# ClimateImpactLab/climate_toolbox

Measured on AMD Instinct MI355X. Metric: gridcell-region-timesteps/sec, higher is better.
Workload: dtype f32

## Files before the change

### climate_toolbox_amd/_lib.py

```python
from __future__ import annotations

import ctypes as C
import os

_HERE = os.path.dirname(os.path.abspath(__file__))
LIB_PATH = os.path.join(_HERE, "lib", "libwagg.so")

EKEY, EINTERNAL = -6, -7
PLAN_NO_LC, PLAN_NO_STREAM, PLAN_NO_LINES, PLAN_LC_MFMA, PLAN_SERIAL_BUILD = 1, 2, 4, 8, 16
FORM_FULL, FORM_TILES, FORM_ENTRIES = 0, 1, 2
FORCE_FORM = {None: 0, "auto": 0, "full": 1, "tiles": 2, "entries": 3}
HOST_PIN, HOST_WHOLE, HOST_LINES, HOST_LINES_WHOLE = 1, 2, 4, 8
DENSE_GENERAL_SORT = 16
GATHER_AUTO, GATHER_RCCL, GATHER_PEER = 0, 1, 2
LAYOUT_TG, LAYOUT_GT = 0, 1
OUT_TR, OUT_RT = 0, 1

EXPORTS = (
    "wagg_version", "wagg_device_count", "wagg_shard_rows", "wagg_last_error", "wagg_profile_enable", "wagg_profile_read",
    "wagg_profile_event_overhead",
    "wagg_resolve_cells", "wagg_backup_fill", "wagg_relabel", "wagg_factorize_i64", "wagg_factorize_bytes",
    "wagg_plan_create", "wagg_plan_destroy", "wagg_plan_get_info", "wagg_plan_get_den", "wagg_plan_status",
    "wagg_apply_f32", "wagg_apply_f64", "wagg_apply_host_f32", "wagg_apply_host_f64",
    "wagg_apply_host_ex_f32", "wagg_apply_host_ex_f64", "wagg_dense_apply_host_f32", "wagg_dense_apply_host_f64",
    "wagg_apply_poly_f32", "wagg_apply_poly_f64", "wagg_apply_edd_f32", "wagg_apply_edd_f64",
    "wagg_apply_poly_host_f32", "wagg_apply_poly_host_f64", "wagg_apply_edd_host_f32", "wagg_apply_edd_host_f64",
    "wagg_gather_f32", "wagg_gather_f64",
    "wagg_transform_poly_f32", "wagg_transform_poly_f64", "wagg_transform_edd_f32", "wagg_transform_edd_f64",
    "wagg_any_less_f32", "wagg_any_less_f64",
    "wagg_dense_create_synth", "wagg_dense_create_host", "wagg_dense_create_from_segments", "wagg_dense_create_synth_blocklocal", "wagg_dense_create_synth_sparse", "wagg_dense_get_info",
    "wagg_dense_destroy", "wagg_dense_clone", "wagg_release_scratch", "wagg_scratch_bytes", "wagg_dense_get_den", "wagg_dense_apply_f32", "wagg_dense_apply_poly_f32",
    "wagg_dense_apply_edd_f32", "wagg_dense_saw_inf",
    "wagg_dense_create_synth_f64", "wagg_dense_create_host_f64", "wagg_dense_create_from_segments_f64",
    "wagg_dense_create_synth_blocklocal_f64", "wagg_dense_apply_f64", "wagg_dense_apply_poly_f64", "wagg_dense_apply_edd_f64",
    "wagg_synth_field_f32", "wagg_synth_field_f64",
    "wagg_apply_host_multi_f32", "wagg_apply_host_multi_f64", "wagg_dense_apply_host_multi_f32", "wagg_dense_apply_host_multi_f64",
    "wagg_host_block_plan", "wagg_host_stats_read",
    "wagg_combine_planes_f32", "wagg_combine_planes_f64", "wagg_take_axis", "wagg_relayout_f32", "wagg_relayout_f64",
    "wagg_dense_create_from_csr", "wagg_dense_create_from_csr_f64", "wagg_synth_table_csr", "wagg_relayout_to_f64", "wagg_upload",
    "wagg_shard_group_create", "wagg_shard_group_destroy", "wagg_shard_group_info",
    "wagg_apply_sharded_f32", "wagg_apply_sharded_f64", "wagg_dense_apply_sharded_f32", "wagg_dense_apply_sharded_f64",
    "wagg_apply", "wagg_struct_size", "wagg_struct_ordinals", "wagg_plan_get_info_sized", "wagg_dense_get_info_sized",
    "wagg_host_stats_read_sized",
    "wagg_plan_create_many", "wagg_plan_many_info", "wagg_plan_get_den_many",
)
STRUCT_PLAN_INFO, STRUCT_DENSE_INFO, STRUCT_HOST_STATS, STRUCT_APPLY_DESC = 0, 1, 2, 3
PLAN_SEGMENT, PLAN_DENSE = 0, 1
SRC_DEVICE, SRC_HOST, SRC_HOST_MULTI, SRC_SHARDED = 0, 1, 2, 3
XF_NONE, XF_POLY, XF_EDD = 0, 1, 2
APPLY_EXACT_F32 = 0x10000
T_F32, T_F64 = 7, 8


class HostStats(C.Structure):
    _fields_ = [(k, C.c_int64) for k in ("calls", "blocks", "registered", "register_failed", "unregistered", "unregister_failed",
                                         "cleanup_failed", "staged_h2d_bytes", "staged_d2h_bytes", "direct_h2d_bytes",
                                         "direct_d2h_bytes", "lines_h2d_bytes", "lines_wait_pack_us", "lines_wait_copy_us", "blocks_retired", "found_page_locked",
                                         "watched_calls", "last_rate_permille")]


def host_stats(reset=False):
    st = HostStats()
    check(load().wagg_host_stats_read_sized(C.byref(st), C.sizeof(st), 1 if reset else 0), "wagg_host_stats_read_sized")
    return {k: int(getattr(st, k)) for k, _ in HostStats._fields_}


def host_block_plan(T, row_bytes, quantum, n_devices=1):
    b, n = C.c_int64(0), C.c_int64(0)
    check(load().wagg_host_block_plan(int(T), int(row_bytes), int(quantum), int(n_devices), C.byref(b), C.byref(n)),
          "wagg_host_block_plan")
    return int(b.value), int(n.value)


class DenseInfo(C.Structure):
    _fields_ = [("G", C.c_int64), ("n_tiles", C.c_int64), ("w_bytes", C.c_int64),
                ("R", C.c_int32), ("n_kt", C.c_int32), ("n_nt", C.c_int32), ("tiled", C.c_int32),
                ("form", C.c_int32), ("elem_bytes", C.c_int32), ("nnz", C.c_int64),
                ("build_s", C.c_double), ("build_upload_s", C.c_double),
                ("est_full_s", C.c_double), ("est_tiles_s", C.c_double), ("est_entries_s", C.c_double), ("walked_entries", C.c_int64),
                ("one_pass_sort", C.c_int32), ("reserved0", C.c_int32)]


class WaggError(RuntimeError):
    pass


class PlanInfo(C.Structure):
    _fields_ = [("nseg_in", C.c_int64), ("nnz", C.c_int64), ("n_groups", C.c_int64),
                ("n_chunks", C.c_int64), ("n_ucells", C.c_int64), ("n_giant", C.c_int64),
                ("n_empty", C.c_int64), ("G", C.c_int64), ("R", C.c_int32), ("lines", C.c_int32),
                ("n_lines128", C.c_int64), ("n_sectors64", C.c_int64), ("n_partial_rows", C.c_int64),
                ("lines_chunks", C.c_int64), ("lines_ucells", C.c_int64), ("lines_lines128", C.c_int64),
                ("n_partial_rows64", C.c_int64), ("lines64_chunks", C.c_int64), ("lines64_ucells", C.c_int64)]


class ApplyDesc(C.Structure):
    _fields_ = [("struct_size", C.c_uint64), ("plan_kind", C.c_int32), ("elem", C.c_int32), ("source", C.c_int32), ("transform", C.c_int32),
                ("plan", C.c_void_p), ("x", C.c_void_p), ("x2", C.c_void_p), ("out", C.c_void_p),
                ("T", C.c_int64), ("ldx", C.c_int64), ("ldo", C.c_int64), ("out_pstride", C.c_int64),
                ("layout", C.c_int32), ("out_layout", C.c_int32), ("offset", C.c_double), ("pow_first", C.c_int32), ("n_pow", C.c_int32),
                ("thresholds", C.c_void_p), ("n_thr", C.c_int32), ("flags", C.c_int32), ("ksplit", C.c_int32), ("n_plans", C.c_int32),
                ("devices", C.c_void_p), ("rows", C.c_void_p), ("group", C.c_void_p), ("root", C.c_int32), ("reserved0", C.c_int32),
                ("stream", C.c_void_p)]


STRUCTS = {STRUCT_PLAN_INFO: PlanInfo, STRUCT_DENSE_INFO: DenseInfo, STRUCT_HOST_STATS: HostStats, STRUCT_APPLY_DESC: ApplyDesc}


def _ptr(v):
    if v is None:
        return None
    if isinstance(v, int):
        return v
    if isinstance(v, C.c_void_p):
        return v.value
    return C.cast(v, C.c_void_p).value


def run(what, **fields):
    d = ApplyDesc()
    d.struct_size = C.sizeof(ApplyDesc)
    d.pow_first = d.n_pow = 1
    for k, v in fields.items():
        setattr(d, k, _ptr(v) if k in _DESC_POINTERS else v)
    check(load().wagg_apply(C.byref(d)), what)


_DESC_POINTERS = frozenset(k for k, t in ApplyDesc._fields_ if t is C.c_void_p)

_lib = None


def load():
    global _lib
    if _lib is not None:
        return _lib
    if not os.path.exists(LIB_PATH):
        raise WaggError(
            "HIP engine not built: %s is missing. Run `python -c \"import __graft_entry__ as g; "
            "g.build()\"` or `make -C climate_toolbox_amd/csrc`. There is no CPU fallback." % LIB_PATH)
    import torch
    L = C.CDLL(LIB_PATH)
    vp, i32p, f64p, f32p = C.c_void_p, C.POINTER(C.c_int32), C.POINTER(C.c_double), C.POINTER(C.c_float)
    L.wagg_version.restype = C.c_int
    L.wagg_shard_rows.argtypes = [C.c_int64, C.c_int, C.c_int, C.POINTER(C.c_int64), C.POINTER(C.c_int64)]
    L.wagg_device_count.restype = C.c_int
    L.wagg_last_error.restype = C.c_char_p
    L.wagg_profile_enable.argtypes = [C.c_int]
    L.wagg_profile_read.argtypes = [f32p, C.c_int, C.POINTER(C.c_int)]
    L.wagg_profile_event_overhead.argtypes = [vp, C.c_int, f32p, f32p]
    u8p, i64p = C.POINTER(C.c_uint8), C.POINTER(C.c_int64)
    L.wagg_resolve_cells.argtypes = [f64p, C.c_int64, f64p, C.c_int64, f64p, f64p, C.c_int64, C.c_int, i32p, i64p]
    L.wagg_backup_fill.argtypes = [f64p, f64p, C.c_int64, f64p]
    L.wagg_relabel.argtypes = [f64p, C.c_int64, C.c_double, C.c_double]
    L.wagg_factorize_i64.argtypes = [i64p, u8p, C.c_int64, i32p, i64p, i64p]
    L.wagg_factorize_bytes.argtypes = [C.c_char_p, C.c_int64, u8p, C.c_int64, i32p, i64p, i64p]
    L.wagg_plan_create.argtypes = [i32p, i32p, f64p, C.c_int64, C.c_int64, C.c_int32, C.c_int64,
                                   C.c_int, C.POINTER(vp)]
    L.wagg_plan_create_many.argtypes = [i32p, i32p, C.POINTER(f64p), C.c_int, C.c_int64, C.c_int64, C.c_int32, C.c_int64,
                                        C.POINTER(i32p), i32p, C.c_int, C.c_int, C.POINTER(vp)]
    L.wagg_plan_many_info.argtypes = [vp, C.POINTER(C.c_int), C.POINTER(C.c_int), i32p, i64p]
    L.wagg_plan_get_den_many.argtypes = [vp, C.c_int, C.c_int, f64p]
    L.wagg_plan_destroy.argtypes = [vp]
    L.wagg_plan_get_info.argtypes = [vp, C.POINTER(PlanInfo)]
    L.wagg_plan_get_info_sized.argtypes = [vp, vp, C.c_uint64]
    L.wagg_dense_get_info_sized.argtypes = [vp, vp, C.c_uint64]
    L.wagg_host_stats_read_sized.argtypes = [vp, C.c_uint64, C.c_int]
    L.wagg_struct_size.argtypes = [C.c_int]
    L.wagg_struct_ordinals.argtypes = [C.c_int, vp, C.c_uint64]
    L.wagg_apply.argtypes = [C.POINTER(ApplyDesc)]
    L.wagg_plan_get_den.argtypes = [vp, f64p]
    L.wagg_plan_status.argtypes = [vp, vp]
    for name in ("wagg_apply_f32", "wagg_apply_f64"):
        getattr(L, name).argtypes = [vp, vp, C.c_int64, C.c_int64, C.c_int, vp, C.c_int64, C.c_int, vp]
    for name in ("wagg_apply_poly_f32", "wagg_apply_poly_f64"):
        getattr(L, name).argtypes = [vp, vp, C.c_int64, C.c_int64, C.c_int, C.c_double, C.c_int, C.c_int, vp,
                                     C.c_int64, C.c_int64, C.c_int, vp]
    for name in ("wagg_apply_poly_host_f32", "wagg_apply_poly_host_f64"):
        getattr(L, name).argtypes = [vp, vp, C.c_int64, C.c_int64, C.c_double, C.c_int, C.c_int, vp, C.c_int64, C.c_int64, C.c_int]
    for name in ("wagg_apply_edd_host_f32", "wagg_apply_edd_host_f64"):
        getattr(L, name).argtypes = [vp, vp, vp, C.c_int64, C.c_int64, C.c_double, f64p, C.c_int, vp, C.c_int64, C.c_int64, C.c_int]
    for name in ("wagg_apply_edd_f32", "wagg_apply_edd_f64"):
        getattr(L, name).argtypes = [vp, vp, vp, C.c_int64, C.c_int64, C.c_int, C.c_double, f64p, C.c_int, vp,
                                     C.c_int64, C.c_int64, C.c_int, vp]
    for name in ("wagg_apply_host_f32", "wagg_apply_host_f64"):
        getattr(L, name).argtypes = [vp, vp, C.c_int64, C.c_int64, C.c_int, vp, C.c_int64, C.c_int]
    for name in ("wagg_apply_host_ex_f32", "wagg_apply_host_ex_f64"):
        getattr(L, name).argtypes = [vp, vp, C.c_int64, C.c_int64, C.c_int, vp, C.c_int64, C.c_int, C.c_int]
    for name in ("wagg_dense_apply_host_f32", "wagg_dense_apply_host_f64"):
        getattr(L, name).argtypes = [vp, vp, C.c_int64, C.c_int64, vp, C.c_int64, C.c_int]
    for name in ("wagg_apply_host_multi_f32", "wagg_apply_host_multi_f64", "wagg_dense_apply_host_multi_f32",
                 "wagg_dense_apply_host_multi_f64"):
        getattr(L, name).argtypes = [C.POINTER(vp), i32p, C.c_int, vp, C.c_int64, C.c_int64, vp, C.c_int64, C.c_int]
    for name in ("wagg_combine_planes_f32", "wagg_combine_planes_f64"):
        getattr(L, name).argtypes = [vp, C.c_int, C.c_int64, f64p, C.c_int64, vp, vp]
    L.wagg_take_axis.argtypes = [vp, C.c_int64, C.c_int64, C.c_int64, vp, C.c_int64, vp, vp]
    for name in ("wagg_relayout_f32", "wagg_relayout_f64"):
        getattr(L, name).argtypes = [vp, C.c_int, C.POINTER(C.c_int64), C.POINTER(C.c_int64), vp, vp]
    L.wagg_relayout_to_f64.argtypes = [vp, C.c_int, C.c_int, C.POINTER(C.c_int64), C.POINTER(C.c_int64), vp, vp]
    L.wagg_upload.argtypes = [vp, vp, C.c_int64]
    L.wagg_host_block_plan.argtypes = [C.c_int64, C.c_int64, C.c_int64, C.c_int, C.POINTER(C.c_int64), C.POINTER(C.c_int64)]
    L.wagg_host_stats_read.argtypes = [C.POINTER(HostStats), C.c_int]
    for name in ("wagg_gather_f32", "wagg_gather_f64"):
        getattr(L, name).argtypes = [vp, C.c_int64, C.c_int64, C.c_int, vp, C.c_int64, vp, C.c_int64,
                                     C.c_int, vp]
    for name in ("wagg_transform_poly_f32", "wagg_transform_poly_f64"):
        getattr(L, name).argtypes = [vp, C.c_int64, C.c_double, C.c_int, vp, vp]
    for name in ("wagg_transform_edd_f32", "wagg_transform_edd_f64"):
        getattr(L, name).argtypes = [vp, vp, C.c_int64, C.c_double, f64p, f64p, C.c_int, vp, vp]
    for name in ("wagg_any_less_f32", "wagg_any_less_f64"):
        getattr(L, name).argtypes = [vp, vp, C.c_int64, C.POINTER(C.c_int), vp]
    L.wagg_dense_create_synth.argtypes = [C.c_int64, C.c_int32, C.c_uint32, C.POINTER(vp)]
    L.wagg_dense_create_host.argtypes = [f32p, C.c_int64, C.c_int32, C.POINTER(vp)]
    L.wagg_dense_create_from_segments.argtypes = [i32p, i32p, f64p, C.c_int64, C.c_int64, C.c_int32, C.c_int,
                                                  C.POINTER(vp)]
    L.wagg_dense_create_synth_blocklocal.argtypes = [C.c_int64, C.c_int32, C.c_uint32, C.c_double, C.POINTER(vp)]
    L.wagg_dense_create_synth_sparse.argtypes = [C.c_int64, C.c_int32, C.c_uint32, C.c_double, C.POINTER(vp)]
    L.wagg_dense_get_info.argtypes = [vp, C.POINTER(DenseInfo)]
    L.wagg_dense_destroy.argtypes = [vp]
    L.wagg_dense_clone.argtypes = [vp, C.c_int, C.POINTER(vp)]
    L.wagg_release_scratch.argtypes = []
    L.wagg_scratch_bytes.argtypes = []
    L.wagg_scratch_bytes.restype = C.c_int64
    L.wagg_dense_get_den.argtypes = [vp, f64p]
    L.wagg_dense_apply_f32.argtypes = [vp, vp, C.c_int64, C.c_int64, vp, C.c_int64, C.c_int, vp]
    L.wagg_dense_apply_poly_f32.argtypes = [vp, vp, C.c_int64, C.c_int64, C.c_double, C.c_int, vp, C.c_int64, C.c_int, vp]
    L.wagg_dense_apply_edd_f32.argtypes = [vp, vp, vp, C.c_int64, C.c_int64, C.c_double, C.c_double, vp, C.c_int64,
                                           C.c_int, vp]
    L.wagg_dense_saw_inf.argtypes = [vp, vp, C.POINTER(C.c_int)]
    L.wagg_dense_create_synth_f64.argtypes = [C.c_int64, C.c_int32, C.c_uint32, C.c_double, C.POINTER(vp)]
    L.wagg_dense_create_synth_blocklocal_f64.argtypes = [C.c_int64, C.c_int32, C.c_uint32, C.c_double, C.POINTER(vp)]
    L.wagg_dense_create_host_f64.argtypes = [f64p, C.c_int64, C.c_int32, C.POINTER(vp)]
    L.wagg_dense_create_from_segments_f64.argtypes = [i32p, i32p, f64p, C.c_int64, C.c_int64, C.c_int32, C.c_int, C.POINTER(vp)]
    for name in ("wagg_dense_create_from_csr", "wagg_dense_create_from_csr_f64"):
        getattr(L, name).argtypes = [i64p, i32p, f64p, C.c_int64, C.c_int32, C.c_int, C.POINTER(vp)]
    L.wagg_synth_table_csr.argtypes = [C.c_int64, C.c_int32, C.c_uint32, C.c_double, C.c_int, i64p, i32p, f64p, C.c_int64, i64p]
    L.wagg_dense_apply_f64.argtypes = [vp, vp, C.c_int64, C.c_int64, vp, C.c_int64, C.c_int, vp]
    L.wagg_dense_apply_poly_f64.argtypes = [vp, vp, C.c_int64, C.c_int64, C.c_double, C.c_int, vp, C.c_int64, C.c_int, vp]
    L.wagg_dense_apply_edd_f64.argtypes = [vp, vp, vp, C.c_int64, C.c_int64, C.c_double, C.c_double, vp, C.c_int64,
                                           C.c_int, vp]
    L.wagg_synth_field_f32.argtypes = [vp, C.c_int64, C.c_int64, C.c_int64, C.c_uint32, C.c_float,
                                       C.c_float, vp]
    L.wagg_synth_field_f64.argtypes = [vp, C.c_int64, C.c_int64, C.c_int64, C.c_uint32, C.c_double,
                                       C.c_double, vp]
    L.wagg_shard_group_create.argtypes = [i32p, C.c_int, C.c_int, C.POINTER(vp)]
    L.wagg_shard_group_destroy.argtypes = [vp]
    L.wagg_shard_group_info.argtypes = [vp, C.POINTER(C.c_int), C.POINTER(C.c_int)]
    for name in ("wagg_apply_sharded_f32", "wagg_apply_sharded_f64", "wagg_dense_apply_sharded_f32", "wagg_dense_apply_sharded_f64"):
        getattr(L, name).argtypes = [vp, C.POINTER(vp), C.POINTER(vp), i64p, C.c_int64, vp, C.c_int64, C.c_int]
    for name in EXPORTS:
        fn = getattr(L, name)
        if name not in ("wagg_last_error", "wagg_scratch_bytes"):
            fn.restype = C.c_int
    _lib = L
    return L


def check(rc, what):
    if rc != 0:
        msg = load().wagg_last_error().decode("utf-8", "replace")
        err = WaggError("%s failed (%d): %s" % (what, rc, msg))
        err.code = int(rc)
        raise err
```

### climate_toolbox_amd/_plans.py

```python
from __future__ import annotations

import os
import threading
from collections import OrderedDict

from ._lib import FORM_ENTRIES, WaggError
from ._memo import _CACHE_LOCK, _fingerprint
from .engine import DensePlan, SparsePlan

_PLAN_CACHE: "OrderedDict[str, SparsePlan]" = OrderedDict()
_PLAN_CACHE_MAX = 8
_PLAN_CACHE_MAX_FRAC = 0.5
_REPLICA_MAX_BYTES = 8 << 30


def _host_devices(setting):
    import torch
    HOST_DEVICES = setting
    if HOST_DEVICES is None:
        return []
    if isinstance(HOST_DEVICES, str):
        if HOST_DEVICES != "all":
            raise ValueError('HOST_DEVICES must be None, "all" or a list of device ordinals')
        if int(os.environ.get("WORLD_SIZE", "1")) > 1:
            return []
        return list(range(torch.cuda.device_count()))
    return [int(d) for d in HOST_DEVICES]


def _host_quantum(plan):
    if isinstance(plan, DensePlan):
        f64 = plan.dtype == "float64"
        if plan.info["form"] == FORM_ENTRIES:
            return 64 if f64 else 128
        return 176 if f64 else 368
    return 64


def _host_replicas(plan, n_rows, row_bytes, setting=None):
    devs = _host_devices(setting)
    if len(devs) < 2 or _plan_bytes(plan) > _REPLICA_MAX_BYTES:
        return ()
    from ._lib import host_block_plan
    if host_block_plan(n_rows, row_bytes, _host_quantum(plan), len(devs))[1] < 2 * len(devs):
        return ()
    own = devs.index(plan.device) if plan.device in devs else 0
    cache = plan.__dict__.setdefault("_replicas", {})
    out = []
    for slot, d in enumerate(devs):
        if slot == own:
            continue
        key = (slot, d)
        if key not in cache:
            cache[key] = plan.replica(d)
        out.append(cache[key])
    return tuple(out)


DENSE_SWITCH = 16.0
_SPARSE_CELLS_PER_S = {True: 2.7e11, False: 1.8e11}
_DENSE_MARGIN = 1.5
_DENSE_BUILD_BYTES_PER_ROW = 64
_ENOMEM = -3


def _dense_floor_s(G, R, nseg, is_f32):
    b = 4 if is_f32 else 8
    n_rb = -(-int(R) // (16 * 43))
    loop = 2.0 * 1.3 * float(nseg) / (30e12 if is_f32 else 13e12)
    pack = 2.0 * b * float(G) / 5.3e12
    return max(b * float(G) * n_rb / 10.1e12, loop) + pack


def _wants_dense(n_ucells, G, layout, R=None, nseg=None, is_f32=True):
    if layout != "TG":
        return False
    if R is None or nseg is None:
        return n_ucells > DENSE_SWITCH * G
    return n_ucells / _SPARSE_CELLS_PER_S[bool(is_f32)] > _DENSE_MARGIN * _dense_floor_s(G, R, nseg, is_f32)


def _dense_bytes(G, R, is_f32=True, nseg=None):
    eb = 4 if is_f32 else 8
    full = eb * ((int(G) + 31) // 32 * 32) * ((int(R) + 255) // 256 * 256)
    if nseg is not None:
        n_buckets = 16 * (-(-int(R) // 688)) * (-(-int(G) // 128))
        return min(full, (64 if is_f32 else 160) * int(nseg) + 7 * (8 if is_f32 else 16) * n_buckets)
    return full


def _prefer_dense(n_ucells, G, R, is_f32, layout, free_bytes, nseg=None):
    return (_wants_dense(n_ucells, G, layout, R=R, nseg=nseg if nseg is not None else n_ucells, is_f32=is_f32)
            and _dense_bytes(G, R, is_f32, nseg=nseg) < 0.6 * free_bytes)


def _plan_bytes(plan):
    return int(plan.info.get("w_bytes", 0)) if isinstance(plan, DensePlan) else 16 * int(plan.info.get("nnz", 0))


def _evict_plans(byte_budget, keep):
    freed = 0
    held = sum(_plan_bytes(p) for p in _PLAN_CACHE.values())
    for key in list(_PLAN_CACHE):
        if not (len(_PLAN_CACHE) > keep or held > max(byte_budget, 0)):
            break
        old = _PLAN_CACHE[key]
        if not old._lease.acquire(blocking=False):
            continue
        try:
            del _PLAN_CACHE[key]
            b = _plan_bytes(old)
            old.close()
        finally:
            old._lease.release()
        held -= b
        freed += b
    return freed


def _drop_plan(plan):
    with _CACHE_LOCK:
        for key, p in list(_PLAN_CACHE.items()):
            if p is plan:
                del _PLAN_CACHE[key]
    plan.close()


_BUILDING = {}


def _plan_for(cell_idx, codes, w_eff, G, R, row_len, is_f32=False, layout="TG", prepared=None):
    if prepared is not None:
        key = prepared.plan_key(cell_idx, G, R, row_len, is_f32, layout)
    else:
        key, _ = _fingerprint(cell_idx, codes, w_eff, extra=repr((int(G), int(R), int(row_len), bool(is_f32), layout)))
    while True:
        with _CACHE_LOCK:
            plan = _PLAN_CACHE.get(key)
            pending = None
            if plan is not None:
                _PLAN_CACHE.move_to_end(key)
            else:
                pending = _BUILDING.get(key)
                if pending is None:
                    _BUILDING[key] = threading.Event()
        if plan is not None:
            plan._lease.acquire()
            if plan._h.value:
                return plan
            plan._lease.release()
            with _CACHE_LOCK:
                if _PLAN_CACHE.get(key) is plan:
                    del _PLAN_CACHE[key]
            continue
        if pending is not None:
            pending.wait()
            continue
        break
    import torch
    plan = None
    try:
        with _CACHE_LOCK:
            free_bytes, total_bytes = torch.cuda.mem_get_info()
            from . import _lib as _libmod
            if _libmod._lib is not None:
                free_bytes += int(_libmod._lib.wagg_scratch_bytes())
            free_bytes += _evict_plans(_PLAN_CACHE_MAX_FRAC * total_bytes, keep=_PLAN_CACHE_MAX - 1)
        need = _dense_bytes(G, R, is_f32, nseg=len(cell_idx)) + _DENSE_BUILD_BYTES_PER_ROW * len(cell_idx)

        def dense_fits():
            nonlocal free_bytes
            if need >= 0.6 * free_bytes:
                with _CACHE_LOCK:
                    free_bytes += _evict_plans(_PLAN_CACHE_MAX_FRAC * total_bytes - need, keep=_PLAN_CACHE_MAX - 1)
            return need < 0.6 * free_bytes

        dt = "float32" if is_f32 else "float64"

        def dense_plan():
            if len(cell_idx) >= 2 ** 31:
                return None
            for attempt in (0, 1):
                try:
                    return DensePlan.from_segments(cell_idx, codes, w_eff, G, R, dtype=dt)
                except WaggError as e:
# ... 80 lines not shown
```

### climate_toolbox_amd/csrc/wagg_common.h

```cpp
#pragma once
#include <hip/hip_runtime.h>
#include <hip/hip_ext.h>
#include <cstdarg>
#include <cstdint>
#include <cstdio>
#include <cstring>
#include <new>
#include <vector>

#include "../../include/wagg.h"

namespace wagg {

void set_error(const char *fmt, ...);

#define WAGG_HIP(expr)                                                                        \
    do {                                                                                      \
        hipError_t e__ = (expr);                                                              \
        if (e__ != hipSuccess) {                                                              \
            wagg::set_error("%s:%d: %s -> %s", __FILE__, __LINE__, #expr,                     \
                            hipGetErrorString(e__));                                          \
            return WAGG_EHIP;                                                                 \
        }                                                                                     \
    } while (0)
// ... 41 lines not shown
    p = __builtin_fmaf(p, az, 0.0010792884277179837f);
    p = __builtin_fmaf(p, az, -0.002406827174127102f);
    p = __builtin_fmaf(p, az, 0.005977150052785873f);
    p = __builtin_fmaf(p, az, -0.022534651681780815f);
    p = __builtin_fmaf(p, az, 0.31830987334251404f);
    const float q = __builtin_amdgcn_sqrtf(t) * t;
    return __builtin_fmaf(w, q * p, __builtin_fmaxf(d, 0.0f));
}
__device__ __forceinline__ double snyder_edd1_finite(double tmin, double tmax, double e) {
    const double M = 0.5 * (tmax + tmin), w = 0.5 * (tmax - tmin);
    const double d = M - e;
    double rw = __builtin_amdgcn_rcp(w);
    rw = __builtin_fma(rw, __builtin_fma(-w, rw, 1.0), rw);
    const double az = __builtin_fmin(__builtin_fabs(d * rw), 1.0);
    const double t = 1.0 - az;
    const double ty = __builtin_amdgcn_rsq(__builtin_fmax(t, 1e-300));
    double st = t * ty;
    st = __builtin_fma(__builtin_fma(-st, st, t), 0.5 * ty, st);
    double p = -8.644295123170258e-07;
    p = __builtin_fma(p, az, 7.147532263874047e-06);
    p = __builtin_fma(p, az, -2.807399717529102e-05);
    p = __builtin_fma(p, az, 7.126284961634285e-05);
    p = __builtin_fma(p, az, -0.0001359898123558899);
    p = __builtin_fma(p, az, 0.0002182750865254441);
    p = __builtin_fma(p, az, -0.0003242640574299061);
    p = __builtin_fma(p, az, 0.000480605991421148);
    p = __builtin_fma(p, az, -0.0007477719612718598);
    p = __builtin_fma(p, az, 0.0012691227365052833);
    p = __builtin_fma(p, az, -0.0024647062510063378);
    p = __builtin_fma(p, az, 0.005985979570242935);
    p = __builtin_fma(p, az, -0.0225351707225776);
    p = __builtin_fma(p, az, 0.3183098861837864);
    return __builtin_fma(w, st * t * p, __builtin_fmax(d, 0.0));
}
template <> __device__ __forceinline__ float snyder_edd1<float>(float tmin, float tmax, float e) {
    const float d = 0.5f * (tmax + tmin) - e;
    const float inner = snyder_edd1_finite(tmin, tmax, e);
    return !(tmin < e) ? d : (!(tmax > e) ? 0.0f : inner);
}

template <typename T> __device__ __forceinline__ T xform1(T x, T off, int pw) {
    const T y = x + off;
    T r = y;
    for (int i = 1; i < pw; ++i) r *= y;
    return r;
}
template <typename V, typename T> __device__ __forceinline__ V xform4(V v, T off, int pw) {
    V r;
#pragma unroll
    for (int c = 0; c < 4; ++c) r[c] = xform1<T>(v[c], off, pw);
    return r;
}

void copy_sized(void *dst, uint64_t dst_size, const void *src, size_t src_size);

hipError_t allow_dynamic_lds(const void *kern, size_t bytes);

bool profile_slot(hipEvent_t *start, hipEvent_t *stop);

inline hipError_t launch_timed_ptr(bool timed, const void *kern, dim3 grid, dim3 block, void **args, size_t shmem, hipStream_t st) {
    hipEvent_t a = nullptr, b = nullptr;
    if (timed && profile_slot(&a, &b)) return hipExtLaunchKernel(kern, grid, block, args, shmem, st, a, b, 0);
    return hipLaunchKernel(kern, grid, block, args, shmem, st);
}
template <typename... Args, typename F = void (*)(Args...)>
inline void launch_timed(bool timed, F kern, dim3 grid, dim3 block, size_t shmem, hipStream_t st, Args... args) {
    hipEvent_t a = nullptr, b = nullptr;
    if (timed && profile_slot(&a, &b)) hipExtLaunchKernelGGL(kern, grid, block, (std::uint32_t)shmem, st, a, b, 0u, args...);
    else hipLaunchKernelGGL(kern, grid, block, shmem, st, args...);
}

hipError_t staged_h2d(void *dst_dev, const void *src_host, size_t bytes, hipStream_t st);
hipError_t staged_d2h_rows(void *dst_host, const void *src_dev, int64_t rows, size_t ld_bytes, size_t row_bytes, hipStream_t st);
inline hipError_t staged_d2h(void *dst_host, const void *src_dev, size_t bytes, hipStream_t st = nullptr) {
    return staged_d2h_rows(dst_host, src_dev, 1, bytes, bytes, st);
}
void clear_error();

hipError_t scratch_alloc(void **p, size_t bytes);
void scratch_free(void *p, bool keep = true);
hipError_t scratch_stream(hipStream_t *st, int role = 0);
void scratch_stream_done(hipStream_t st, int role = 0, bool keep = true);
void release_scratch(int what = 7);
template <typename T>
struct ScratchBuf {
    T *p = nullptr;
    ScratchBuf() = default;
    ScratchBuf(const ScratchBuf &) = delete;
    ScratchBuf &operator=(const ScratchBuf &) = delete;
    hipError_t alloc(size_t count) { return scratch_alloc(reinterpret_cast<void **>(&p), (count ? count : 1) * sizeof(T)); }
    ~ScratchBuf() { if (p) { (void)hipDeviceSynchronize(); scratch_free(p); } }
};

template <typename T>
struct DevBuf {
    T *p = nullptr;
    size_t n = 0;
    DevBuf() = default;
    DevBuf(const DevBuf &) = delete;
    DevBuf &operator=(const DevBuf &) = delete;
    ~DevBuf() { if (p) (void)hipFree(p); }
    hipError_t alloc(size_t count) {
        if (p) { (void)hipFree(p); p = nullptr; }
        n = count;
        hipError_t e = hipMalloc((void **)&p, (count ? count : 1) * sizeof(T));
        if (e == hipErrorOutOfMemory) {
            (void)hipGetLastError();
            release_scratch();
            e = hipMalloc((void **)&p, (count ? count : 1) * sizeof(T));
        }
        return e;
    }
    hipError_t upload(const std::vector<T> &h, hipStream_t st = nullptr) {
        hipError_t e = alloc(h.size());
        if (e != hipSuccess || h.empty()) return e;
        return staged_h2d(p, h.data(), h.size() * sizeof(T), st);
    }
};

}
```

### climate_toolbox_amd/csrc/wagg_dense.hip

```cpp
#include <algorithm>
#include <cfloat>
#include <chrono>
#include <cmath>
#include <limits>
#include <cstdlib>
#include <type_traits>

#include "wagg_dense_int.h"
#include "wagg_entry.h"

namespace wagg {

constexpr int D_MT = 23;
constexpr int D_BN = 256;
constexpr int D_ROWB = 128;
constexpr int D_THREADS = 512;
constexpr int D_WTB = D_BN * D_ROWB;
constexpr int D_WSLOTS = D_WTB / 16;
static_assert(D_WTB / 1024 == 32, "4 one-KiB W pieces per wave");
constexpr int d_xt_bytes(int mt) { return mt * 16 * D_ROWB; }
constexpr int d_buf_bytes(int mt) { return d_xt_bytes(mt) + D_WTB; }
static_assert(2 * d_buf_bytes(D_MT) <= 160 * 1024, "LDS budget");

typedef float f32x4 __attribute__((ext_vector_type(4)));
typedef double f64x2 __attribute__((ext_vector_type(2)));
typedef double f64x4 __attribute__((ext_vector_type(4)));
typedef const void __attribute__((address_space(1))) *gptr_t;
typedef void __attribute__((address_space(3))) *lptr_t;

template <typename T> struct DT;
template <> struct DT<float> {
    typedef f32x4 vec;
    typedef f32x4 acc;
    static constexpr int EPP = 4, BK = 32, MT_MAX = 23;
    static __device__ __forceinline__ acc mfma(float a, float b, acc c) { return __builtin_amdgcn_mfma_f32_16x16x4f32(a, b, c, 0, 0, 0); }
    static __device__ __forceinline__ int crow(int kq, int reg) { return kq * 4 + reg; }
};
template <> struct DT<double> {
    typedef f64x2 vec;
    typedef f64x4 acc;
    static constexpr int EPP = 2, BK = 16, MT_MAX = 11;
    static __device__ __forceinline__ acc mfma(double a, double b, acc c) { return __builtin_amdgcn_mfma_f64_16x16x4f64(a, b, c, 0, 0, 0); }
    static __device__ __forceinline__ int crow(int kq, int reg) { return kq + 4 * reg; }
};

__host__ __device__ __forceinline__ int tile_slot(int row, int p) { return row * 8 + (p ^ ((row >> 1) & 7)); }

template <typename T, int DBG = 0, bool TILED = false, int MT = D_MT, bool RM = false>
__global__ __launch_bounds__(D_THREADS, 2) void dense_mfma_kernel(
    const T *__restrict__ Xp, const T *__restrict__ Wp, int n_kt, int n_nt, int n_mb, int S,
    int kt_per_slice, T *__restrict__ slabs, const int32_t *__restrict__ tile_kt = nullptr,
    const int32_t *__restrict__ tile_off = nullptr, int64_t ldxB = 0, int Tn = 0, const int *__restrict__ gate = nullptr) {
#define WAGG_PIECES 0
#include "wagg_dense_kernel.inc"
#undef WAGG_PIECES
}

template <typename T, int MT, bool RM>
__global__ __launch_bounds__(D_THREADS, 2) void dense_pieces_kernel(
    const T *__restrict__ Xp, const T *__restrict__ Wp, int n_kt, int n_nt, int n_mb, int S,
    int kt_per_slice, T *__restrict__ slabs, const int32_t *__restrict__ tile_kt, const int32_t *__restrict__ tile_off,
    int64_t ldxB, int Tn, const int *__restrict__ gate) {
    constexpr bool TILED = true;
    constexpr int DBG = 0;
    (void)n_kt; (void)n_mb; (void)S; (void)kt_per_slice;
#define WAGG_PIECES 1
#include "wagg_dense_kernel.inc"
#undef WAGG_PIECES
}

template <typename T>
__global__ void dense_pack_x_kernel(const T *__restrict__ X, int64_t Tn, int64_t ldx, int64_t G,
                                    int n_kt, int bm, int64_t n_slots, int aligned, typename DT<T>::vec *__restrict__ Xp,
                                    PackXfT<T> xf, int *__restrict__ inf_flag, const int *__restrict__ gate = nullptr) {
    typedef typename DT<T>::vec vec_t;
    constexpr int E = DT<T>::EPP;
    if (gate != nullptr && *gate == 0) return;
    const int64_t stride = (int64_t)gridDim.x * blockDim.x;
    const int tile_slots = bm * 8;
    bool inf_seen = false;
    for (int64_t s = (int64_t)blockIdx.x * blockDim.x + threadIdx.x; s < n_slots; s += stride) {
        const int slot = (int)(s % tile_slots);
        const int64_t tk = s / tile_slots;
// ... 608 lines not shown
#else
    (void)fill_all;
#endif
    int rc = dense_alloc<T>(G, R, out, tiled ? (int64_t)tiles.size() : -1, entries);
    if (rc != WAGG_OK) return rc;
    wagg_dense *d = *out;
    WAGG_BUILD_STAMP(ctx, "plan alloc");
    auto fail = [&](int code) { (void)ctx.sync(); delete d; *out = nullptr; return code; };
    if (entries) {
        ctx.release_to(0);
        rc = spmm_build_from_sorted<T>(ctx, d, se);
        if (rc != WAGG_OK) return fail(rc);
    } else {
        hipError_t e = hipMemsetAsync(d->W.p, 0, 16 * (size_t)d->w_slots(), ctx.st);
        if (e == hipSuccess && tiled) e = dense_set_tiles(d, tiles, nullptr, ctx.st);
        if (e == hipSuccess && tiled) {
            word_rank = ctx.take<uint32_t>((size_t)n_words);
            e = word_rank ? staged_h2d(word_rank, hrank.data(), sizeof(uint32_t) * hrank.size(), ctx.st) : hipErrorOutOfMemory;
        }
        if (e == hipSuccess && se.n_u > 0) {
            hipLaunchKernelGGL((table_scatter_kernel<T>), dim3(nblk), dim3(256), 0, ctx.st, (const uint64_t *)se.key.p, (const double *)se.w.p,
                               se.n_u, kg, n_kt, (const uint32_t *)bitmap, (const uint32_t *)word_rank, reinterpret_cast<T *>(d->W.p));
            e = hipGetLastError();
        }
        if (e != hipSuccess) { set_error("densify: %s", hipGetErrorString(e)); return fail(WAGG_EHIP); }
    }
    hipError_t e = hipMemcpyAsync(d->den64.p, se.den.p, sizeof(double) * (size_t)R, hipMemcpyDeviceToDevice, ctx.st);
    if (e != hipSuccess) { set_error("densify den: %s", hipGetErrorString(e)); return fail(WAGG_EHIP); }
    rc = dense_den_to_host(d, ctx.st);
    if (rc == WAGG_OK) rc = dense_finish_scales(d, ctx.st);
    if (rc != WAGG_OK) return fail(rc);
    e = ctx.sync();
    if (e != hipSuccess) { set_error("plan build: %s", hipGetErrorString(e)); return fail(WAGG_EHIP); }
    WAGG_BUILD_STAMP(ctx, "pack + den to host");
    if (entries) d->sp.nnz = se.n_u;
    d->nnz_table = se.n_u;
    d->est_row_s[0] = cost.t_full; d->est_row_s[1] = cost.t_tiled; d->est_row_s[2] = cost.t_entries;
    d->walked_entries = walked;
    d->one_pass_sort = se.chunkwise;
    d->build.upload_s = t_up;
    d->build.total_s = wall_s() - t0;
    d->build.device_s = d->build.total_s - t_up;
    return WAGG_OK;
}

template <typename T, bool TILED, int MT, bool RM = false>
static const void *mfma_kernel_ptr() {
    if constexpr (TILED) return (const void *)dense_pieces_kernel<T, MT, RM>;
    else return (const void *)dense_mfma_kernel<T, 0, false, MT, RM>;
}
template <typename T>
static const void *pick_full_rm_kernel(int MT, bool rm) {
#define WAGG_PICK(M) case M: return rm ? (const void *)dense_mfma_kernel<T, 0, false, M, true> \
                                       : (const void *)dense_mfma_kernel<T, 256, false, M, false>
    if constexpr (sizeof(T) == 4) {
        switch (MT) { WAGG_PICK(20); WAGG_PICK(21); WAGG_PICK(22); WAGG_PICK(23); default: return nullptr; }
    } else {
        switch (MT) { WAGG_PICK(10); WAGG_PICK(11); default: return nullptr; }
    }
#undef WAGG_PICK
}

template <typename T>
static const void *pick_mfma_kernel(int MT, bool tiled, bool rm = false) {
#define WAGG_PICK(M) case M: return tiled ? (rm ? mfma_kernel_ptr<T, true, M, true>() : mfma_kernel_ptr<T, true, M>()) \
                                          : mfma_kernel_ptr<T, false, M>()
    if constexpr (sizeof(T) == 4) {
        switch (MT) {
            WAGG_PICK(1); WAGG_PICK(2); WAGG_PICK(3); WAGG_PICK(4); WAGG_PICK(5); WAGG_PICK(6); WAGG_PICK(8);
            WAGG_PICK(10); WAGG_PICK(12); WAGG_PICK(14); WAGG_PICK(16); WAGG_PICK(18); WAGG_PICK(20);
            WAGG_PICK(21); WAGG_PICK(22); WAGG_PICK(23);
            default: return nullptr;
        }
    } else {
        switch (MT) {
            WAGG_PICK(1); WAGG_PICK(2); WAGG_PICK(3); WAGG_PICK(4); WAGG_PICK(5); WAGG_PICK(6); WAGG_PICK(8);
            WAGG_PICK(10); WAGG_PICK(11);
            default: return nullptr;
        }
    }
#undef WAGG_PICK
}

static const void *pick_split_kernel(int MT) {
#define WAGG_PICK(M) case M: return (const void *)dense_split_kernel<M>
    switch (MT) {
        WAGG_PICK(1); WAGG_PICK(2); WAGG_PICK(3); WAGG_PICK(4); WAGG_PICK(5); WAGG_PICK(6); WAGG_PICK(8);
        WAGG_PICK(10); WAGG_PICK(12); WAGG_PICK(14); WAGG_PICK(16); WAGG_PICK(18); WAGG_PICK(20);
        WAGG_PICK(21); WAGG_PICK(22); WAGG_PICK(23);
        default: return nullptr;
    }
#undef WAGG_PICK
}

static int dense_apply_split(wagg_dense *d, const float *X_dev, int64_t Tn, int64_t ldx, const PackXfT<float> &xf,
                             float *out_dev, int64_t ldo, int MT, int n_mb, int S, hipStream_t st) {
    const int n_nt = d->n_nt, n_kt = d->n_kt, bm = MT * 16;
    const int kt_per_slice = (n_kt + S - 1) / S;
    const int64_t nblk = (int64_t)n_nt * n_mb * S;
    WAGG_REQUIRE(nblk < (int64_t)0x7fffffff, "grid too large");
    const void *kern = pick_split_kernel(MT);
    if (!kern) { set_error("no split kernel for MT=%d", MT); return WAGG_EINVAL; }
    const size_t need = (size_t)nblk * bm * D_BN;
    if (d->slabs.n < need) WAGG_HIP(d->slabs.alloc(need));
    const int64_t x_slots = (int64_t)n_mb * n_kt * bm * 8;
    if (d->xp.n < (size_t)x_slots * 4) WAGG_HIP(d->xp.alloc((size_t)x_slots * 4));
    if (d->xmax.n < (size_t)Tn) WAGG_HIP(d->xmax.alloc((size_t)Tn));
    const int aligned = ((ldx * sizeof(float)) % 16 == 0) && ((reinterpret_cast<uintptr_t>(X_dev) & 15) == 0) &&
                        (xf.mode != XF_EDD || (reinterpret_cast<uintptr_t>(xf.X2) & 15) == 0);
#ifdef WAGG_DIAG
    if (const char *dbg = MT == D_MT ? getenv("WAGG_SPLIT_DBG") : nullptr) {
        switch (atoi(dbg)) {
            case 1: kern = (const void *)dense_split_kernel<D_MT, 1>; break;
            case 4: kern = (const void *)dense_split_kernel<D_MT, 4>; break;
            case 5: kern = (const void *)dense_split_kernel<D_MT, 5>; break;
            case 8: kern = (const void *)dense_split_kernel<D_MT, 8>; break;
            case 9: kern = (const void *)dense_split_kernel<D_MT, 9>; break;
            default: break;
        }
    }
#endif
    const size_t shmem = 3 * (size_t)d_xt_bytes(MT);
    WAGG_HIP(allow_dynamic_lds(kern, shmem));
    unsigned *xmax = reinterpret_cast<unsigned *>(d->xmax.p);
    WAGG_HIP(hipMemsetAsync(xmax, 0, sizeof(unsigned) * (size_t)Tn, st));
    const int64_t gx = (d->G + 4095) / 4096 < 64 ? (d->G + 4095) / 4096 : 64;
    hipLaunchKernelGGL(dense_rowmax_kernel, dim3((unsigned)gx, (unsigned)Tn), dim3(256), 0, st, X_dev, ldx, d->G, xf, xmax);
    hipLaunchKernelGGL(dense_pack_x_split_kernel, dim3(256 * 16), dim3(256), 0, st, X_dev, Tn, ldx, d->G, n_kt, bm, x_slots, aligned,
                       (const unsigned *)xmax, reinterpret_cast<f16x8 *>(d->xp.p), xf, d->inf_dev);
    WAGG_HIP(hipGetLastError());
    const f16x8 *xp = reinterpret_cast<const f16x8 *>(d->xp.p);
    const float *wp = d->W.p, *wmax = d->wmax.p;
    float *slabs = d->slabs.p;
    int n_kt_a = n_kt, n_nt_a = n_nt, n_mb_a = n_mb, S_a = S, kps = kt_per_slice;
    void *args[] = {&xp, &wp, &wmax, &n_kt_a, &n_nt_a, &n_mb_a, &S_a, &kps, &slabs};
    WAGG_HIP(launch_timed_ptr(true, kern, dim3((unsigned)nblk), dim3(D_THREADS), args, shmem, st));
    hipLaunchKernelGGL(dense_reduce_split_kernel, dim3((unsigned)((d->R + 255) / 256), (unsigned)Tn), dim3(256), 0, st,
                       (const float *)slabs, n_nt, S, bm, d->R, (const float *)d->den32.p, (const unsigned *)xmax, wmax, out_dev, ldo);
    WAGG_HIP(hipGetLastError());
    return WAGG_OK;
}

template <typename T>
static int dense_apply(wagg_dense *d, const T *X_dev, int64_t Tn, int64_t ldx, const PackXfT<T> &xf,
                       T *out_dev, int64_t ldo, int ksplit, void *stream, bool exact = false) {
    typedef typename DT<T>::vec vec_t;
    WAGG_REQUIRE(d != nullptr, "dense plan is NULL");
    WAGG_REQUIRE(d->f64 == (sizeof(T) == 8), "this plan holds %s weights: use the matching wagg_dense_apply_*",
                 d->f64 ? "fp64" : "fp32");
    WAGG_REQUIRE(Tn >= 0, "T < 0");
    if (Tn == 0) return WAGG_OK;
    WAGG_REQUIRE(X_dev && out_dev, "X/out is NULL");
    WAGG_REQUIRE(xf.mode != XF_EDD || xf.X2 != nullptr, "tasmax is NULL");
    WAGG_REQUIRE(ldx >= d->G && ldo >= d->R, "ldx/ldo too small");
    WAGG_REQUIRE(ksplit >= 0 && ksplit % 8 == 0, "ksplit must be 0 or a multiple of 8");
    if (d->spmm) return spmm_apply<T>(d, X_dev, Tn, ldx, xf, out_dev, ldo, (hipStream_t)stream);
    constexpr int64_t ROWS_MAX = (int64_t)(65535 / (DT<T>::MT_MAX * 16)) * (DT<T>::MT_MAX * 16);
    if (Tn > ROWS_MAX) {
        for (int64_t t0 = 0; t0 < Tn; t0 += ROWS_MAX) {
            PackXfT<T> xg = xf;
            if (xg.X2) xg.X2 += t0 * ldx;
            const int64_t rows = Tn - t0 < ROWS_MAX ? Tn - t0 : ROWS_MAX;
            if (int rc = dense_apply<T>(d, X_dev + t0 * ldx, rows, ldx, xg, out_dev + t0 * ldo, ldo, ksplit, stream, exact)) return rc;
        }
        return WAGG_OK;
    }
    const int n_nt = d->n_nt, n_kt = d->n_kt;
    constexpr int BM_MAX = DT<T>::MT_MAX * 16;
    const int n_mb = (int)((Tn + BM_MAX - 1) / BM_MAX);
    const int rows = (int)((Tn + n_mb - 1) / n_mb);
    static const int mts32[] = {1, 2, 3, 4, 5, 6, 8, 10, 12, 14, 16, 18, 20, 21, 22, 23};
    static const int mts64[] = {1, 2, 3, 4, 5, 6, 8, 10, 11};
    int MT = DT<T>::MT_MAX;
    if constexpr (sizeof(T) == 4) { for (int m : mts32) if (m * 16 >= rows) { MT = m; break; } }
    else { for (int m : mts64) if (m * 16 >= rows) { MT = m; break; } }
    const int bm = MT * 16;
    if (n_mb >= 2) {
        const int64_t head = (int64_t)(n_mb - 1) * bm, tail = Tn - head;
        if (tail > 0) {
            int MT_tail = DT<T>::MT_MAX;
            if constexpr (sizeof(T) == 4) { for (int m : mts32) if ((int64_t)m * 16 >= tail) { MT_tail = m; break; } }
            else { for (int m : mts64) if ((int64_t)m * 16 >= tail) { MT_tail = m; break; } }
            if (MT_tail >= 4 && MT - MT_tail >= 2) {
                PackXfT<T> xt = xf;
                if (xt.X2) xt.X2 += head * ldx;
                if (int rc = dense_apply<T>(d, X_dev, head, ldx, xf, out_dev, ldo, ksplit, stream, exact)) return rc;
                return dense_apply<T>(d, X_dev + head * ldx, tail, ldx, xt, out_dev + head * ldo, ldo, ksplit, stream, exact);
            }
        }
    }
    int S = ksplit ? ksplit : pick_ksplit((int64_t)n_nt * n_mb, n_kt);
    if constexpr (sizeof(T) == 4) {
        if (!d->tiled && !exact && d->wmax.p != nullptr) return dense_apply_split(d, X_dev, Tn, ldx, xf, out_dev, ldo, MT, n_mb, S, (hipStream_t)stream);
    }
    const wagg_dense::TilePieces *tp = nullptr;
    if (d->tiled) {
        if (int rc = tile_pieces_for(d, n_mb, (hipStream_t)stream, &tp)) return rc;
        S = 1;
    }
    const int kt_per_slice = (n_kt + S - 1) / S;
    const int64_t nblk = tp ? (int64_t)tp->n_wg : (int64_t)n_nt * n_mb * S;
    WAGG_REQUIRE(nblk < (int64_t)0x7fffffff, "grid too large");
    const size_t n_slabs = tp ? (size_t)tp->n_slabs : (size_t)n_nt * n_mb * S;
    const size_t need = (n_slabs ? n_slabs : 1) * bm * D_BN * (sizeof(T) / 4);
    if (d->slabs.n < need) WAGG_HIP(d->slabs.alloc(need));
    const int64_t x_slots = (int64_t)n_mb * n_kt * bm * 8;
    if (d->xp.n < (size_t)x_slots * 4) WAGG_HIP(d->xp.alloc((size_t)x_slots * 4));
    const int aligned = ((ldx * sizeof(T)) % 16 == 0) && ((reinterpret_cast<uintptr_t>(X_dev) & 15) == 0) &&
                        (xf.mode != XF_EDD || (reinterpret_cast<uintptr_t>(xf.X2) & 15) == 0);
    const size_t shmem = 2 * (size_t)d_buf_bytes(MT);
    hipStream_t st = (hipStream_t)stream;
    const void *kern = pick_mfma_kernel<T>(MT, d->tiled);
    if (!kern) { set_error("no kernel for MT=%d", MT); return WAGG_EINVAL; }
    bool rm = xf.mode == 0 && aligned && d->G % DT<T>::BK == 0 && ((volatile int *)d->inf_host)[1] == 0;
    const void *kern_rm = nullptr;
// ... 62 lines not shown

template <typename T>
static int apply_poly(wagg_dense *d, const T *X_dev, int64_t Tn, int64_t ldx, double offset, int power, T *out_dev,
                      int64_t ldo, int ksplit, void *stream, bool exact = false) {
    WAGG_REQUIRE(power >= 1 && power <= 16, "power must lie in [1, 16], got %d", power);
    PackXfT<T> xf;
    xf.mode = power; xf.off = (T)offset;
    return dense_apply<T>(d, X_dev, Tn, ldx, xf, out_dev, ldo, ksplit, stream, exact);
}

template <typename T>
static int apply_edd(wagg_dense *d, const T *tasmin, const T *tasmax, int64_t Tn, int64_t ldx, double offset,
                     double threshold, T *out_dev, int64_t ldo, int ksplit, void *stream, bool exact = false) {
    PackXfT<T> xf;
    xf.mode = XF_EDD; xf.off = (T)offset; xf.thr = (T)threshold; xf.X2 = tasmax;
    return dense_apply<T>(d, tasmin, Tn, ldx, xf, out_dev, ldo, ksplit, stream, exact);
}

}

extern "C" int wagg_dense_create_synth(int64_t G, int32_t R, uint32_t seed, wagg_dense **out) {
    return wagg::create_synth<float>(G, R, seed, 1.0, out);
}
extern "C" int wagg_dense_create_synth_sparse(int64_t G, int32_t R, uint32_t seed, double fill, wagg_dense **out) {
    return wagg::create_synth<float>(G, R, seed, fill, out);
}
extern "C" int wagg_dense_create_synth_f64(int64_t G, int32_t R, uint32_t seed, double fill, wagg_dense **out) {
    return wagg::create_synth<double>(G, R, seed, fill, out);
}
extern "C" int wagg_dense_create_synth_blocklocal(int64_t G, int32_t R, uint32_t seed, double fill, wagg_dense **out) {
    return wagg::create_synth_blocklocal<float>(G, R, seed, fill, out);
}
extern "C" int wagg_dense_create_synth_blocklocal_f64(int64_t G, int32_t R, uint32_t seed, double fill, wagg_dense **out) {
    return wagg::create_synth_blocklocal<double>(G, R, seed, fill, out);
}
extern "C" int wagg_dense_create_host(const float *W_host, int64_t G, int32_t R, wagg_dense **out) {
    return wagg::create_host<float>(W_host, G, R, out);
}
extern "C" int wagg_dense_create_host_f64(const double *W_host, int64_t G, int32_t R, wagg_dense **out) {
    return wagg::create_host<double>(W_host, G, R, out);
}
extern "C" int wagg_dense_create_from_segments(const int32_t *cell_idx, const int32_t *region_code,
                                               const double *w_eff, int64_t nseg, int64_t G, int32_t R,
                                               int flags, wagg_dense **out) {
    return wagg::create_from_table<float>(cell_idx, nullptr, region_code, w_eff, nseg, G, R, flags, out);
}
extern "C" int wagg_dense_create_from_segments_f64(const int32_t *cell_idx, const int32_t *region_code,
                                                   const double *w_eff, int64_t nseg, int64_t G, int32_t R,
                                                   int flags, wagg_dense **out) {
    return wagg::create_from_table<double>(cell_idx, nullptr, region_code, w_eff, nseg, G, R, flags, out);
}

extern "C" int wagg_dense_create_from_csr(const int64_t *rowptr, const int32_t *col, const double *val, int64_t G, int32_t R,
                                          int flags, wagg_dense **out) {
    using namespace wagg;
    WAGG_REQUIRE(rowptr != nullptr, "rowptr is NULL");
    return create_from_table<float>(nullptr, rowptr, col, val, 0, G, R, flags, out);
}
extern "C" int wagg_dense_create_from_csr_f64(const int64_t *rowptr, const int32_t *col, const double *val, int64_t G, int32_t R,
                                              int flags, wagg_dense **out) {
    using namespace wagg;
    WAGG_REQUIRE(rowptr != nullptr, "rowptr is NULL");
    return create_from_table<double>(nullptr, rowptr, col, val, 0, G, R, flags, out);
}

extern "C" int wagg_dense_get_info_sized(const wagg_dense *d, void *info_buf, uint64_t size) {
    using namespace wagg;
    WAGG_REQUIRE(d && info_buf, "NULL argument");
    wagg_dense_info st;
    std::memset(&st, 0, sizeof(st));
    wagg_dense_info *info = &st;
    info->G = d->G; info->R = d->R; info->n_kt = d->n_kt; info->n_nt = d->n_nt;
    info->n_tiles = d->n_tiles; info->tiled = d->tiled ? 1 : 0;
    info->w_bytes = d->spmm ? (int64_t)d->sp.n_groups * 4 * (d->f64 ? wagg::SpT<double>::GW : wagg::SpT<float>::GW) : d->w_slots() * 16;
    info->form = d->spmm ? WAGG_FORM_ENTRIES : (d->tiled ? WAGG_FORM_TILES : WAGG_FORM_FULL);
    info->elem_bytes = d->f64 ? 8 : 4;
    info->nnz = d->spmm ? d->sp.nnz : d->nnz_table;
    info->build_s = d->build.total_s;
    info->build_upload_s = d->build.upload_s;
    for (int k = 0; k < 3; ++k) info->est_row_s[k] = d->est_row_s[k];
    info->walked_entries = d->walked_entries;
    info->one_pass_sort = d->one_pass_sort ? 1 : 0;
    info->reserved0 = 0;
    copy_sized(info_buf, size, &st, sizeof(st));
    return WAGG_OK;
}
extern "C" int wagg_dense_get_info(const wagg_dense *d, wagg_dense_info *info) {
    return wagg_dense_get_info_sized(d, info, sizeof(wagg_dense_info));
}

namespace wagg {
template <typename E>
static hipError_t clone_buf(DevBuf<E> &dst, int dst_dev, const DevBuf<E> &src, int src_dev) {
    if (!src.p) return hipSuccess;
    hipError_t e = dst.alloc(src.n);
    if (e == hipSuccess && src.n) e = hipMemcpyPeer(dst.p, dst_dev, src.p, src_dev, src.n * sizeof(E));
    return e;
}
}

extern "C" int wagg_dense_clone(const wagg_dense *src, int device, wagg_dense **out) {
    using namespace wagg;
    clear_error();
    WAGG_REQUIRE(out != nullptr, "out is NULL");
    *out = nullptr;
    WAGG_REQUIRE(src != nullptr, "dense plan is NULL");
    int n_dev = 0, cur = 0;
    WAGG_HIP(hipGetDeviceCount(&n_dev));
    WAGG_REQUIRE(device >= 0 && device < n_dev, "no device %d (%d visible)", device, n_dev);
    WAGG_HIP(hipGetDevice(&cur));
    wagg_dense *d = new (std::nothrow) wagg_dense();
    if (!d) { set_error("host allocation failed"); return WAGG_ENOMEM; }
    hipError_t e = hipSetDevice(device);
    try {
        d->G = src->G; d->R = src->R; d->n_kt = src->n_kt; d->n_nt = src->n_nt; d->f64 = src->f64;
        d->tiled = src->tiled; d->n_tiles = src->n_tiles; d->spmm = src->spmm;
        d->sp.rw = src->sp.rw; d->sp.n_rb = src->sp.n_rb; d->sp.n_chunks = src->sp.n_chunks;
        d->sp.nnz = src->sp.nnz; d->sp.n_groups = src->sp.n_groups;
        d->nnz_table = src->nnz_table; d->walked_entries = src->walked_entries; d->one_pass_sort = src->one_pass_sort;
        for (int k = 0; k < 3; ++k) d->est_row_s[k] = src->est_row_s[k];
        d->den_host = src->den_host;
        d->nt_first = src->nt_first;
        d->device = device;
        const double t0 = wall_s();
        if (e == hipSuccess) e = hipDeviceGetAttribute(&d->ncu, hipDeviceAttributeMultiprocessorCount, device);
        if (e == hipSuccess) e = d->nonfinite.alloc(1);
        if (e == hipSuccess) e = hipHostMalloc((void **)&d->inf_host, 2 * sizeof(int), hipHostMallocMapped);
        if (e == hipSuccess) { d->inf_host[0] = d->inf_host[1] = 0; e = hipHostGetDevicePointer((void **)&d->inf_dev, d->inf_host, 0); }
        if (e == hipSuccess) e = clone_buf(d->W, device, src->W, src->device);
        if (e == hipSuccess) e = clone_buf(d->den32, device, src->den32, src->device);
        if (e == hipSuccess) e = clone_buf(d->den64, device, src->den64, src->device);
        if (e == hipSuccess) e = clone_buf(d->wmax, device, src->wmax, src->device);
        if (e == hipSuccess) e = clone_buf(d->tile_kt, device, src->tile_kt, src->device);
        if (e == hipSuccess) e = clone_buf(d->sp.ent, device, src->sp.ent, src->device);
        if (e == hipSuccess) e = clone_buf(d->sp.grp_off, device, src->sp.grp_off, src->device);
        if (e == hipSuccess) e = hipStreamSynchronize(nullptr);
        d->build.total_s = d->build.device_s = wall_s() - t0;
    } catch (const std::bad_alloc &) {
        (void)hipSetDevice(cur);
        delete d;
        set_error("host allocation failed");
        return WAGG_ENOMEM;
    }
    const hipError_t back = hipSetDevice(cur);
    if (e != hipSuccess || back != hipSuccess) {
        set_error("clone of a dense plan onto device %d: %s", device, hipGetErrorString(e != hipSuccess ? e : back));
        delete d;
        return e == hipErrorOutOfMemory ? WAGG_ENOMEM : WAGG_EHIP;
    }
    *out = d;
    return WAGG_OK;
}

extern "C" int wagg_dense_destroy(wagg_dense *d) {
    delete d;
    return WAGG_OK;
}

extern "C" int wagg_dense_get_den(const wagg_dense *d, double *den_host) {
    using namespace wagg;
    WAGG_REQUIRE(d && den_host, "NULL argument");
    std::memcpy(den_host, d->den_host.data(), sizeof(double) * (size_t)d->R);
    return WAGG_OK;
}

int wagg::entry::dense_apply_f32(wagg_dense *d, const float *X_dev, int64_t T, int64_t ldx,
                                    float *out_dev, int64_t ldo, int ksplit, void *stream, bool exact) {
    return wagg::dense_apply<float>(d, X_dev, T, ldx, wagg::PackXfT<float>{}, out_dev, ldo, ksplit, stream, exact);
}
int wagg::entry::dense_apply_f64(wagg_dense *d, const double *X_dev, int64_t T, int64_t ldx,
                                    double *out_dev, int64_t ldo, int ksplit, void *stream) {
    return wagg::dense_apply<double>(d, X_dev, T, ldx, wagg::PackXfT<double>{}, out_dev, ldo, ksplit, stream);
}
int wagg::entry::dense_apply_poly_f32(wagg_dense *d, const float *X_dev, int64_t T, int64_t ldx, double offset,
                                         int power, float *out_dev, int64_t ldo, int ksplit, void *stream, bool exact) {
    return wagg::apply_poly<float>(d, X_dev, T, ldx, offset, power, out_dev, ldo, ksplit, stream, exact);
}
int wagg::entry::dense_apply_poly_f64(wagg_dense *d, const double *X_dev, int64_t T, int64_t ldx, double offset,
                                         int power, double *out_dev, int64_t ldo, int ksplit, void *stream) {
    return wagg::apply_poly<double>(d, X_dev, T, ldx, offset, power, out_dev, ldo, ksplit, stream);
}
int wagg::entry::dense_apply_edd_f32(wagg_dense *d, const float *tasmin_dev, const float *tasmax_dev, int64_t T,
                                        int64_t ldx, double offset, double threshold, float *out_dev, int64_t ldo,
                                        int ksplit, void *stream, bool exact) {
    return wagg::apply_edd<float>(d, tasmin_dev, tasmax_dev, T, ldx, offset, threshold, out_dev, ldo, ksplit, stream, exact);
}
int wagg::entry::dense_apply_edd_f64(wagg_dense *d, const double *tasmin_dev, const double *tasmax_dev, int64_t T,
                                        int64_t ldx, double offset, double threshold, double *out_dev, int64_t ldo,
                                        int ksplit, void *stream) {
    return wagg::apply_edd<double>(d, tasmin_dev, tasmax_dev, T, ldx, offset, threshold, out_dev, ldo, ksplit, stream);
}

namespace wagg {
static int check_dense_device(const wagg_dense *d) {
    int cur = 0;
    WAGG_HIP(hipGetDevice(&cur));
    WAGG_REQUIRE(cur == d->device, "the dense plan was created on device %d, the current device is %d", d->device, cur);
    return WAGG_OK;
}

template <typename T>
static int dense_apply_host(wagg_dense *d, const T *X_host, int64_t Tn, int64_t ldx, T *out_host, int64_t ldo, int flags,
                            bool exact = false) {
    clear_error();
    WAGG_REQUIRE(d != nullptr, "dense plan is NULL");
    WAGG_REQUIRE(Tn >= 0, "T < 0");
    if (Tn == 0) return WAGG_OK;
    WAGG_REQUIRE(X_host && out_host, "X/out is NULL");
    WAGG_REQUIRE(ldx >= d->G && ldo >= d->R, "ldx/ldo too small");
    WAGG_REQUIRE((flags & ~(WAGG_HOST_PIN | WAGG_HOST_WHOLE)) == 0, "unknown host flags 0x%x", flags);
    if (int rc = check_dense_device(d)) return rc;
    if (flags & WAGG_HOST_WHOLE) {
        ScratchBuf<T> dx, dout;
        WAGG_HIP(dx.alloc((size_t)(Tn * ldx)));
        WAGG_HIP(dout.alloc((size_t)(Tn * ldo)));
        const bool pin = (flags & WAGG_HOST_PIN) != 0;
        if (int rc = copy_to_device(dx.p, X_host, sizeof(T) * (size_t)((Tn - 1) * ldx + d->G), pin)) return rc;
        const int rc = dense_apply<T>(d, dx.p, Tn, ldx, PackXfT<T>{}, dout.p, ldo, 0, nullptr, exact);
        if (rc != WAGG_OK) return rc;
        WAGG_HIP(hipDeviceSynchronize());
        return copy_rows_to_host(out_host, dout.p, Tn, sizeof(T) * (size_t)ldo, sizeof(T) * (size_t)d->R, pin);
    }
    return stream_host_rows<T>(X_host, Tn, ldx, d->G, out_host, ldo, d->R, flags, d->spmm ? SpT<T>::TB : DT<T>::MT_MAX * 16, 1, nullptr,
                               [&](int, const T *xd, int64_t rows, T *od, hipStream_t st) {
                                   return dense_apply<T>(d, xd, rows, ldx, PackXfT<T>{}, od, ldo, 0, (void *)st, exact);
                               },
                               [](int, hipStream_t) {});
}

template <typename T>
static int dense_apply_host_multi(wagg_dense *const *plans, const int *devices, int n, const T *X_host, int64_t Tn, int64_t ldx,
                                  T *out_host, int64_t ldo, int flags) {
    clear_error();
    WAGG_REQUIRE(plans && devices && n >= 1 && n <= 64, "need 1..64 plan replicas and their devices");
    WAGG_REQUIRE((flags & ~WAGG_HOST_PIN) == 0, "unknown host flags 0x%x", flags);
    WAGG_REQUIRE(Tn >= 0, "T < 0");
// ... 51 lines not shown
```

### climate_toolbox_amd/csrc/wagg_dense_int.h

```cpp
#pragma once
#include <memory>

#include "wagg_build.h"
#include "wagg_host.h"

namespace wagg {

template <typename T> struct PackXfT {
    int mode = 0;
    T off = T(0), thr = T(0);
    const T *X2 = nullptr;
};
typedef PackXfT<float> PackXf;

template <typename T>
__device__ __forceinline__ T pack_xf(const PackXfT<T> &xf, T x, T x2, bool &inf_seen) {
    T y = x;
    if (xf.mode > 0) y = xform1<T>(x, xf.off, xf.mode);
    else if (xf.mode == XF_EDD) y = snyder_edd1<T>(x + xf.off, x2 + xf.off, xf.thr);
    inf_seen |= __builtin_isinf(y);
    return y == y ? y : T(0);
}

constexpr int SP_WAVES = 16;
constexpr int SP_THREADS = SP_WAVES * 64;
constexpr int SP_ROW = 512;
constexpr int SP_KC = 128;
constexpr int SP_ACC = 88;
constexpr int SP_RW_MAX = SP_ACC / 2 - 1;
constexpr int SP_TRASH = 2 * SP_RW_MAX;
constexpr int SP_GROUP = 8;
constexpr int SP_PAD_GROUPS = 48;
template <typename T> struct SpT {
    static constexpr int TB = SP_ROW / (int)sizeof(T);
    static constexpr int GW = 4 + 8 * (int)(sizeof(T) / 4);
    static constexpr int WSLOT = 128 * (int)sizeof(T);
};
__host__ __device__ inline unsigned sp_entry_lo(int cell_in_chunk, int j) { return (unsigned)(cell_in_chunk << 9 | 2 * j); }
template <typename T> __host__ __device__ inline int64_t sp_lo16_index(int64_t pos) {
    return (pos >> 3) * (2 * SpT<T>::GW) + (pos & 7);
}
template <typename T> __host__ __device__ inline int64_t sp_w_index(int64_t pos) {
    return (pos >> 3) * SpT<T>::GW + 4 + (pos & 7) * (int)(sizeof(T) / 4);
}

struct SpmmPlan {
    int rw = 0;
    int n_rb = 0;
    int n_chunks = 0;
    int64_t nnz = 0, n_groups = 0;
    DevBuf<uint32_t> ent;
    DevBuf<int32_t> grp_off;
};

}

struct wagg_dense {
    int64_t G = 0;
    int32_t R = 0;
    int n_kt = 0, n_nt = 0;
    bool f64 = false;
    wagg::DevBuf<float> W, den32, slabs, xp;
    wagg::DevBuf<double> den64;
    wagg::DevBuf<float> wmax, xmax;
    std::vector<double> den_host;
    bool tiled = false;
    int64_t n_tiles = 0;
    wagg::DevBuf<int32_t> tile_kt;
    std::vector<int32_t> nt_first;
    struct TilePieces {
        int n_mb = 0, n_wg = 0, n_slabs = 0;
        wagg::DevBuf<int32_t> tab;
        int64_t slab_first_at = 0;
    };
    std::vector<std::unique_ptr<TilePieces>> pieces;
    int64_t w_slots() const { return n_tiles * (8192 / 4); }
    bool spmm = false;
    wagg::SpmmPlan sp;
    int ncu = 256;
    int device = 0;
    int *inf_host = nullptr, *inf_dev = nullptr;
    wagg::DevBuf<int> nonfinite;
    int64_t nnz_table = -1;
    wagg::BuildTimes build;
    double est_row_s[3] = {0, 0, 0};
    int64_t walked_entries = 0;
    bool one_pass_sort = false;
    ~wagg_dense() { if (inf_host) wagg::note_cleanup(hipHostFree(inf_host), "hipHostFree(inf note)"); }
};

namespace wagg {
template <typename T> int spmm_build_synth(wagg_dense *d, uint32_t seed, double fill);
void spmm_geometry(int64_t G, int32_t R, SpmmPlan &sp);
template <typename T> int spmm_build_from_sorted(BuildCtx &ctx, wagg_dense *d, const SortedEntries &se);
int spmm_list_cost(BuildCtx &ctx, const SortedEntries &se, int64_t *walked_entries);
template <typename T> int spmm_apply(wagg_dense *d, const T *X, int64_t Tn, int64_t ldx, const PackXfT<T> &xf, T *out,
                                     int64_t ldo, hipStream_t stream);
int dense_alloc_common(wagg_dense *d);
}
```

### climate_toolbox_amd/csrc/wagg_dense_split.inc

```
typedef _Float16 f16x8 __attribute__((ext_vector_type(8)));

__host__ __device__ __forceinline__ int split_exp(float m) {
    int e = 0;
    if (!(m > 0.0f)) return 0;
    (void)frexpf(m, &e);
    return 15 - e;
}

typedef _Float16 f16x2 __attribute__((ext_vector_type(2)));
typedef unsigned u32x4 __attribute__((ext_vector_type(4)));
__device__ __forceinline__ void split_w8(f32x4 a, f32x4 b, int e, f16x8 &hi, f16x8 &lo) {
    u32x4 H, L;
#pragma unroll
    for (int p = 0; p < 4; ++p) {
        const float v0 = __builtin_amdgcn_ldexpf(p < 2 ? a[2 * p] : b[2 * p - 4], e);
        const float v1 = __builtin_amdgcn_ldexpf(p < 2 ? a[2 * p + 1] : b[2 * p - 3], e);
        const unsigned h = __builtin_bit_cast(unsigned, f16x2{(_Float16)v0, (_Float16)v1});
        unsigned l;
        asm("v_fma_mixlo_f16 %0, %1, -1.0, %2 op_sel_hi:[1,0,0]\n\t"
            "v_fma_mixhi_f16 %0, %1, -1.0, %3 op_sel:[1,0,0] op_sel_hi:[1,0,0]\n\t"
            "s_nop 1"
            : "=&v"(l) : "v"(h), "v"(v0), "v"(v1));
        H[p] = h;
        L[p] = l;
    }
    hi = __builtin_bit_cast(f16x8, H);
    lo = __builtin_bit_cast(f16x8, L);
}


__device__ __forceinline__ __amdgpu_buffer_rsrc_t split_tile_rsrc(const char *base, int bytes) {
    const uint64_t a = reinterpret_cast<uint64_t>(base);
    const uint64_t u = (uint64_t)(uint32_t)__builtin_amdgcn_readfirstlane((unsigned)a) |
                       (uint64_t)(uint32_t)__builtin_amdgcn_readfirstlane((unsigned)(a >> 32)) << 32;
    return __builtin_amdgcn_make_buffer_rsrc(reinterpret_cast<void *>(u), (short)0, bytes, 0x00020000);
}

template <int MT, int DBG = 0>
__global__ __launch_bounds__(D_THREADS, 2) void dense_split_kernel(
    const f16x8 *__restrict__ Xp, const float *__restrict__ Wp, const float *__restrict__ wmax, int n_kt, int n_nt, int n_mb,
    int S, int kt_per_slice, float *__restrict__ slabs) {
    static_assert(MT <= D_MT, "accumulators of MT row blocks must fit the register file");
    extern __shared__ __attribute__((aligned(16))) char lds[];
    constexpr int XT4 = d_xt_bytes(MT);
    constexpr int XPIECES = XT4 / 1024;
    constexpr int NXP = (XPIECES + 7) / 8;
    static_assert(NXP <= 6, "at most six X pieces per wave");
    constexpr int VM_KEEP = 4 + NXP;
    constexpr int WAIT_TILE = (VM_KEEP & 15) | (7 << 4) | (0 << 8) | ((VM_KEEP >> 4) << 14);

    const int tid = threadIdx.x;
    const int lane = tid & 63;
    const int wave = __builtin_amdgcn_readfirstlane(tid >> 6);
    const int lr = lane & 15, kq = lane >> 4;

    int j = (int)(blockIdx.x >> 3);
    const int nt = j % n_nt; j /= n_nt;
    const int mb = j % n_mb;
    const int ks = (int)(blockIdx.x & 7) + 8 * (j / n_mb);
    const int kt0 = ks * kt_per_slice;
    const int kt1 = kt0 + kt_per_slice < n_kt ? kt0 + kt_per_slice : n_kt;
    const int ntiles = kt1 > kt0 ? kt1 - kt0 : 0;
    const int64_t w_first = (int64_t)nt * n_kt + kt0;
    const int ew0 = split_exp(wmax[nt * D_BN + wave * 32 + lr]);
    const int ew1 = split_exp(wmax[nt * D_BN + wave * 32 + 16 + lr]);

    const int f = lr >> 1;
    const unsigned frag0 = (lr * 8 + (kq ^ f)) * 16;
    const unsigned frag1 = (lr * 8 + ((kq ^ f) ^ 4)) * 16;
    const char *xslice = reinterpret_cast<const char *>(Xp) + ((int64_t)mb * n_kt + kt0) * XT4;
    const char *wslice = reinterpret_cast<const char *>(Wp) + w_first * D_WTB;
    const unsigned lane16 = lane * 16;
    const unsigned wfrag0 = wave * 4096 + frag0, wfrag1 = wave * 4096 + frag1;
#define WAGG_RSRC(base, bytes) split_tile_rsrc(base, bytes)
#define WAGG_DMA_X(i, xr, buf)                                                                    \
    do {                                                                                          \
        constexpr int i_ = (i);                                                                   \
        const int q_ = (wave + 8 * i_) % XPIECES;                                                 \
        __builtin_amdgcn_raw_ptr_buffer_load_lds(xr, (lptr_t)(lds + (buf) * XT4 + q_ * 1024), 16, lane16, q_ * 1024, 0, 0); \
    } while (0)
#define WAGG_DMA_XALL(tile, buf)                                                                  \
    do {                                                                                          \
        const auto xr_ = WAGG_RSRC(xslice + (int64_t)(tile) * XT4, XT4);                          \
        WAGG_DMA_X(0, xr_, buf);                                                                  \
        if constexpr (NXP > 1) WAGG_DMA_X(NXP > 1 ? 1 : 0, xr_, buf);                             \
        if constexpr (NXP > 2) WAGG_DMA_X(NXP > 2 ? 2 : 0, xr_, buf);                             \
        if constexpr (NXP > 3) WAGG_DMA_X(NXP > 3 ? 3 : 0, xr_, buf);                             \
        if constexpr (NXP > 4) WAGG_DMA_X(NXP > 4 ? 4 : 0, xr_, buf);                             \
        if constexpr (NXP > 5) WAGG_DMA_X(NXP > 5 ? 5 : 0, xr_, buf);                             \
    } while (0)
#define WAGG_LOAD_W(tile)                                                                         \
    do {                                                                                          \
        const auto wr_ = WAGG_RSRC(wslice + (int64_t)(tile) * D_WTB, D_WTB);                      \
        b00 = __builtin_bit_cast(f32x4, __builtin_amdgcn_raw_buffer_load_b128(wr_, wfrag0, 0, 0));        \
        b01 = __builtin_bit_cast(f32x4, __builtin_amdgcn_raw_buffer_load_b128(wr_, wfrag1, 0, 0));        \
        b10 = __builtin_bit_cast(f32x4, __builtin_amdgcn_raw_buffer_load_b128(wr_, wfrag0 + 2048, 0, 0)); \
        b11 = __builtin_bit_cast(f32x4, __builtin_amdgcn_raw_buffer_load_b128(wr_, wfrag1 + 2048, 0, 0)); \
    } while (0)

    f32x4 acc[MT][2];
#pragma unroll
    for (int m = 0; m < MT; ++m) acc[m][0] = acc[m][1] = f32x4{0, 0, 0, 0};

    f32x4 b00, b01, b10, b11;
    if (ntiles > 0) {
        const int t1 = ntiles > 1 ? 1 : 0;
        WAGG_LOAD_W(0);
        WAGG_DMA_XALL(0, 0);
        WAGG_DMA_XALL(t1, 1);
        asm volatile("s_waitcnt vmcnt(0)" ::: "memory");
        __builtin_amdgcn_s_barrier();
    }

#define WAGG_SPLIT(A, B, E, HI, LO)                                                               \
    do {                                                                                          \
        if constexpr (DBG & 8) { HI = __builtin_bit_cast(f16x8, A); LO = __builtin_bit_cast(f16x8, B); } \
        else split_w8(A, B, E, HI, LO);                                                           \
    } while (0)
#define WAGG_MFMA16(RB, CB, A, B) acc[RB][CB] = __builtin_amdgcn_mfma_f32_16x16x32_f16(A, B, acc[RB][CB], 0, 0, 0)
#define WAGG_READ_A(H, L, RB)                                                                     \
    do {                                                                                          \
        H = *reinterpret_cast<const f16x8 *>(img + frag0 + (RB) * 2048);                          \
        L = *reinterpret_cast<const f16x8 *>(img + frag1 + (RB) * 2048);                          \
    } while (0)
    constexpr auto xdma_block = [](int i) { return MT <= 2 ? MT - 1 : 2 + i * (MT - 2) / NXP; };
#define WAGG_DMA_AT(RB, i)                                                                        \
    do {                                                                                          \
        if constexpr (!(DBG & 1) && (i) < NXP && xdma_block(i) == (RB)) WAGG_DMA_X((i) < NXP ? (i) : 0, xfar, bfar); \
    } while (0)
#define WAGG_DMA_BLOCK(RB)                                                                        \
    do {                                                                                          \
        WAGG_DMA_AT(RB, 0); WAGG_DMA_AT(RB, 1); WAGG_DMA_AT(RB, 2);                               \
        WAGG_DMA_AT(RB, 3); WAGG_DMA_AT(RB, 4); WAGG_DMA_AT(RB, 5);                               \
    } while (0)
#define WAGG_BLOCK_(RB, H, L, NH, NL)                                                             \
    do {                                                                                          \
        __builtin_amdgcn_sched_barrier(0);                                                        \
        WAGG_MFMA16(RB, 0, H, wl0);                                                               \
        __builtin_amdgcn_sched_barrier(0);                                                        \
        if constexpr ((RB) + 1 < MT) WAGG_READ_A(NH, NL, (RB) + 1 < MT ? (RB) + 1 : 0);           \
        __builtin_amdgcn_sched_barrier(0);                                                        \
        WAGG_MFMA16(RB, 1, H, wl1);                                                               \
        WAGG_MFMA16(RB, 0, L, wh0);                                                               \
        WAGG_MFMA16(RB, 1, L, wh1);                                                               \
        WAGG_MFMA16(RB, 0, H, wh0);                                                               \
        WAGG_MFMA16(RB, 1, H, wh1);                                                               \
        __builtin_amdgcn_sched_barrier(0);                                                        \
        WAGG_DMA_BLOCK(RB);                                                                       \
    } while (0)
#define WAGG_BLOCK(RB)                                                                            \
    do {                                                                                          \
        if constexpr ((RB) < MT) {                                                                \
            constexpr int rb_ = (RB) < MT ? (RB) : 0;                                             \
            if constexpr ((RB) & 1) WAGG_BLOCK_(rb_, aBh, aBl, aAh, aAl);                         \
            else WAGG_BLOCK_(rb_, aAh, aAl, aBh, aBl);                                            \
        }                                                                                         \
    } while (0)

    int bcur = 0;
    for (int tile = 0; tile < ntiles; ++tile) {
        const char *img = lds + bcur * XT4;
        const int bfar = bcur == 0 ? 2 : bcur - 1;
        const int tnext = tile + 1 < ntiles ? tile + 1 : ntiles - 1;
        const int tfar = tile + 2 < ntiles ? tile + 2 : ntiles - 1;
        const auto xfar = WAGG_RSRC(xslice + (int64_t)tfar * XT4, XT4);
        f16x8 wh0, wl0, wh1, wl1, aAh, aAl, aBh, aBl;
        WAGG_READ_A(aAh, aAl, 0);
        WAGG_SPLIT(b00, b01, ew0, wh0, wl0);
        if constexpr (MT > 1) WAGG_READ_A(aBh, aBl, MT > 1 ? 1 : 0);
        __builtin_amdgcn_sched_barrier(0);
        WAGG_MFMA16(0, 0, aAh, wl0);
        WAGG_MFMA16(0, 0, aAl, wh0);
        WAGG_MFMA16(0, 0, aAh, wh0);
        if constexpr (MT > 1) {
            WAGG_MFMA16(MT > 1 ? 1 : 0, 0, aBh, wl0);
            WAGG_MFMA16(MT > 1 ? 1 : 0, 0, aBl, wh0);
            WAGG_MFMA16(MT > 1 ? 1 : 0, 0, aBh, wh0);
        }
        WAGG_SPLIT(b10, b11, ew1, wh1, wl1);
        __builtin_amdgcn_sched_barrier(0);
        if constexpr (!(DBG & 1)) WAGG_LOAD_W(tnext);
        __builtin_amdgcn_sched_barrier(0);
        WAGG_MFMA16(0, 1, aAh, wl1);
        WAGG_MFMA16(0, 1, aAl, wh1);
        WAGG_MFMA16(0, 1, aAh, wh1);
        __builtin_amdgcn_sched_barrier(0);
        if constexpr (MT > 2) WAGG_READ_A(aAh, aAl, MT > 2 ? 2 : 0);
        __builtin_amdgcn_sched_barrier(0);
        if constexpr (MT > 1) {
            WAGG_MFMA16(MT > 1 ? 1 : 0, 1, aBh, wl1);
            WAGG_MFMA16(MT > 1 ? 1 : 0, 1, aBl, wh1);
            WAGG_MFMA16(MT > 1 ? 1 : 0, 1, aBh, wh1);
        }
        __builtin_amdgcn_sched_barrier(0);
        WAGG_DMA_BLOCK(0); WAGG_DMA_BLOCK(1);
        WAGG_BLOCK(2); WAGG_BLOCK(3); WAGG_BLOCK(4); WAGG_BLOCK(5);
        WAGG_BLOCK(6); WAGG_BLOCK(7); WAGG_BLOCK(8); WAGG_BLOCK(9); WAGG_BLOCK(10); WAGG_BLOCK(11);
        WAGG_BLOCK(12); WAGG_BLOCK(13); WAGG_BLOCK(14); WAGG_BLOCK(15); WAGG_BLOCK(16); WAGG_BLOCK(17);
        WAGG_BLOCK(18); WAGG_BLOCK(19); WAGG_BLOCK(20); WAGG_BLOCK(21); WAGG_BLOCK(22);
        static_assert(MT <= 23, "row blocks are written out up to 22");
        __builtin_amdgcn_sched_barrier(0);
        if constexpr (!(DBG & 4)) {
            __builtin_amdgcn_s_waitcnt(WAIT_TILE);
            __builtin_amdgcn_s_barrier();
        }
        bcur = bcur == 2 ? 0 : bcur + 1;
    }
    asm volatile("s_waitcnt vmcnt(0)" ::: "memory");

    float *slab = slabs + ((((int64_t)mb * n_nt + nt) * S + ks) * (MT * 16)) * D_BN;
#pragma unroll
    for (int m = 0; m < MT; ++m)
#pragma unroll
        for (int cb = 0; cb < 2; ++cb)
#pragma unroll
            for (int r = 0; r < 4; ++r)
                slab[(m * 16 + kq * 4 + r) * D_BN + wave * 32 + cb * 16 + lr] = acc[m][cb][r];
#undef WAGG_RSRC
#undef WAGG_DMA_X
#undef WAGG_DMA_XALL
#undef WAGG_LOAD_W
#undef WAGG_DMA_AT
#undef WAGG_DMA_BLOCK
#undef WAGG_SPLIT
#undef WAGG_MFMA16
#undef WAGG_READ_A
#undef WAGG_BLOCK_
#undef WAGG_BLOCK
}

__global__ void dense_rowmax_kernel(const float *__restrict__ X, int64_t ldx, int64_t G, PackXfT<float> xf,
                                    unsigned *__restrict__ rowmax) {
    const int64_t t = blockIdx.y;
    const float *src = X + t * ldx;
    const float *src2 = xf.mode == XF_EDD ? xf.X2 + t * ldx : src;
    bool inf_seen = false;
    float m = 0.0f;
    for (int64_t g = (int64_t)blockIdx.x * blockDim.x + threadIdx.x; g < G; g += (int64_t)gridDim.x * blockDim.x) {
        const float y = pack_xf<float>(xf, src[g], src2[g], inf_seen);
        const float a = fabsf(y);
        m = a <= FLT_MAX && a > m ? a : m;
    }
#pragma unroll
    for (int o = 32; o >= 1; o >>= 1) m = fmaxf(m, __shfl_xor(m, o, 64));
    __shared__ float wm[16];
    if ((threadIdx.x & 63) == 0) wm[threadIdx.x >> 6] = m;
    __syncthreads();
    if (threadIdx.x == 0) {
        for (int w = 1; w < (int)(blockDim.x >> 6); ++w) m = fmaxf(m, wm[w]);
        if (m > 0.0f) atomicMax(rowmax + t, __float_as_uint(m));
    }
}

__global__ void dense_pack_x_split_kernel(const float *__restrict__ X, int64_t Tn, int64_t ldx, int64_t G, int n_kt, int bm,
                                          int64_t n_slots, int aligned, const unsigned *__restrict__ rowmax,
                                          f16x8 *__restrict__ Xp, PackXfT<float> xf, int *__restrict__ inf_flag) {
    const int64_t stride = (int64_t)gridDim.x * blockDim.x;
    const int tile_slots = bm * 8;
    bool inf_seen = false;
    for (int64_t s = (int64_t)blockIdx.x * blockDim.x + threadIdx.x; s < n_slots; s += stride) {
        const int slot = (int)(s % tile_slots);
        const int64_t tk = s / tile_slots;
        const int kt = (int)(tk % n_kt);
        const int64_t mb = tk / n_kt;
        const int row = slot >> 3, p = (slot & 7) ^ ((row >> 1) & 7);
        const bool low = p >= 4;
        const int64_t t = mb * bm + row, k0 = (int64_t)kt * 32 + 4 * (p & 3);
        f16x8 o;
#pragma unroll
        for (int c = 0; c < 8; ++c) o[c] = (_Float16)0.0f;
        if (t < Tn) {
            const int ex = split_exp(__uint_as_float(rowmax[t]));
            const float *src = X + t * ldx;
            const float *src2 = xf.mode == XF_EDD ? xf.X2 + t * ldx : src;
            float v[8], h[8];
#pragma unroll
            for (int c = 0; c < 8; ++c) { v[c] = 0.0f; h[c] = 0.0f; }
#pragma unroll
            for (int half = 0; half < 2; ++half) {
                const int64_t kk = k0 + 16 * half;
                if (aligned && kk + 4 <= G) {
                    const f32x4 a = *reinterpret_cast<const f32x4 *>(src + kk);
                    const f32x4 b = xf.mode == XF_EDD ? *reinterpret_cast<const f32x4 *>(src2 + kk) : a;
#pragma unroll
                    for (int c = 0; c < 4; ++c) { v[4 * half + c] = a[c]; h[4 * half + c] = b[c]; }
                } else {
#pragma unroll
                    for (int c = 0; c < 4; ++c) if (kk + c < G) { v[4 * half + c] = src[kk + c]; h[4 * half + c] = src2[kk + c]; }
                }
            }
#pragma unroll
            for (int c = 0; c < 8; ++c) {
                const int64_t k = k0 + 16 * (c >> 2) + (c & 3);
                if (k >= G) continue;
                const float y = __builtin_amdgcn_ldexpf(pack_xf<float>(xf, v[c], h[c], inf_seen), ex);
                const _Float16 hi = (_Float16)y;
                o[c] = low ? (__builtin_isinf(y) ? (_Float16)0.0f : (_Float16)(y - (float)hi)) : hi;
            }
        }
        Xp[s] = o;
    }
    if (inf_seen) __hip_atomic_store(inf_flag, 1, __ATOMIC_RELAXED, __HIP_MEMORY_SCOPE_SYSTEM);
}

__global__ void dense_reduce_split_kernel(const float *__restrict__ slabs, int n_nt, int S, int bm, int32_t R,
                                          const float *__restrict__ den, const unsigned *__restrict__ rowmax,
                                          const float *__restrict__ wmax, float *__restrict__ out, int64_t ldo) {
    const int64_t r = (int64_t)blockIdx.x * blockDim.x + threadIdx.x;
    const int64_t t = blockIdx.y;
    if (r >= R) return;
    const int mb = (int)(t / bm), tl = (int)(t % bm);
// ... 26 lines not shown
```

### climate_toolbox_amd/csrc/wagg_desc.hip

```cpp
#include <cstddef>
#include <cstring>
#include <type_traits>

#include "wagg_common.h"
#include "wagg_dense_int.h"
#include "wagg_entry.h"
#include "wagg_host.h"
#include "wagg_sparse_int.h"

namespace wagg {
namespace {

const char *src_name(int s) {
    switch (s) {
        case WAGG_SRC_DEVICE: return "device";
        case WAGG_SRC_HOST: return "host";
        case WAGG_SRC_HOST_MULTI: return "host-multi";
        case WAGG_SRC_SHARDED: return "sharded";
        default: return "?";
    }
}
const char *xf_name(int x) { return x == WAGG_XF_NONE ? "none" : x == WAGG_XF_POLY ? "poly" : x == WAGG_XF_EDD ? "edd" : "?"; }

int unsupported(const wagg_apply_desc &d, const char *why) {
// ... 282 lines not shown
extern "C" int wagg_dense_apply_f64(wagg_dense *p, const double *X_dev, int64_t T, int64_t ldx, double *out_dev, int64_t ldo, int ksplit, void *stream) {
    wagg_apply_desc d = base(DEN, F64, WAGG_SRC_DEVICE, p, X_dev, T, ldx, out_dev, ldo);
    d.ksplit = ksplit; d.stream = stream;
    return wagg_apply(&d);
}
extern "C" int wagg_dense_apply_poly_f32(wagg_dense *p, const float *X_dev, int64_t T, int64_t ldx, double offset, int power, float *out_dev, int64_t ldo,
                                         int ksplit, void *stream) {
    wagg_apply_desc d = base(DEN, F32, WAGG_SRC_DEVICE, p, X_dev, T, ldx, out_dev, ldo);
    d.ksplit = ksplit; d.stream = stream;
    return wagg_apply(&poly(d, offset, power, 1, 0));
}
extern "C" int wagg_dense_apply_poly_f64(wagg_dense *p, const double *X_dev, int64_t T, int64_t ldx, double offset, int power, double *out_dev, int64_t ldo,
                                         int ksplit, void *stream) {
    wagg_apply_desc d = base(DEN, F64, WAGG_SRC_DEVICE, p, X_dev, T, ldx, out_dev, ldo);
    d.ksplit = ksplit; d.stream = stream;
    return wagg_apply(&poly(d, offset, power, 1, 0));
}
extern "C" int wagg_dense_apply_edd_f32(wagg_dense *p, const float *tasmin_dev, const float *tasmax_dev, int64_t T, int64_t ldx, double offset,
                                        double threshold, float *out_dev, int64_t ldo, int ksplit, void *stream) {
    wagg_apply_desc d = base(DEN, F32, WAGG_SRC_DEVICE, p, tasmin_dev, T, ldx, out_dev, ldo);
    d.ksplit = ksplit; d.stream = stream;
    return wagg_apply(&edd(d, tasmax_dev, offset, &threshold, 1, 0));
}
extern "C" int wagg_dense_apply_edd_f64(wagg_dense *p, const double *tasmin_dev, const double *tasmax_dev, int64_t T, int64_t ldx, double offset,
                                        double threshold, double *out_dev, int64_t ldo, int ksplit, void *stream) {
    wagg_apply_desc d = base(DEN, F64, WAGG_SRC_DEVICE, p, tasmin_dev, T, ldx, out_dev, ldo);
    d.ksplit = ksplit; d.stream = stream;
    return wagg_apply(&edd(d, tasmax_dev, offset, &threshold, 1, 0));
}
extern "C" int wagg_dense_apply_host_f32(wagg_dense *p, const float *X_host, int64_t T, int64_t ldx, float *out_host, int64_t ldo, int flags) {
    wagg_apply_desc d = base(DEN, F32, WAGG_SRC_HOST, p, X_host, T, ldx, out_host, ldo);
    d.flags = flags;
    return wagg_apply(&d);
}
extern "C" int wagg_dense_apply_host_f64(wagg_dense *p, const double *X_host, int64_t T, int64_t ldx, double *out_host, int64_t ldo, int flags) {
    wagg_apply_desc d = base(DEN, F64, WAGG_SRC_HOST, p, X_host, T, ldx, out_host, ldo);
    d.flags = flags;
    return wagg_apply(&d);
}
extern "C" int wagg_dense_apply_host_multi_f32(wagg_dense *const *plans, const int *devices, int n_devices, const float *X_host, int64_t T, int64_t ldx,
                                               float *out_host, int64_t ldo, int flags) {
    wagg_apply_desc d = base(DEN, F32, WAGG_SRC_HOST_MULTI, plans, X_host, T, ldx, out_host, ldo);
    d.devices = devices; d.n_plans = n_devices; d.flags = flags;
    return wagg_apply(&d);
}
extern "C" int wagg_dense_apply_host_multi_f64(wagg_dense *const *plans, const int *devices, int n_devices, const double *X_host, int64_t T, int64_t ldx,
                                               double *out_host, int64_t ldo, int flags) {
    wagg_apply_desc d = base(DEN, F64, WAGG_SRC_HOST_MULTI, plans, X_host, T, ldx, out_host, ldo);
    d.devices = devices; d.n_plans = n_devices; d.flags = flags;
    return wagg_apply(&d);
}
extern "C" int wagg_dense_apply_sharded_f32(wagg_shard_group *g, wagg_dense *const *plans, const float *const *X_dev, const int64_t *rows, int64_t ldx,
                                            float *out_root, int64_t ldo, int root) {
    wagg_apply_desc d = base(DEN, F32, WAGG_SRC_SHARDED, plans, X_dev, 0, ldx, out_root, ldo);
    d.group = g; d.rows = rows; d.root = root;
    return wagg_apply(&d);
}
extern "C" int wagg_dense_apply_sharded_f64(wagg_shard_group *g, wagg_dense *const *plans, const double *const *X_dev, const int64_t *rows, int64_t ldx,
                                            double *out_root, int64_t ldo, int root) {
    wagg_apply_desc d = base(DEN, F64, WAGG_SRC_SHARDED, plans, X_dev, 0, ldx, out_root, ldo);
    d.group = g; d.rows = rows; d.root = root;
    return wagg_apply(&d);
}
#undef SEG
#undef DEN
#undef F32
#undef F64

namespace wagg {
namespace {
template <typename F> void put(int &k, F &f) {
    ++k;
    if constexpr (std::is_pointer_v<F>) f = reinterpret_cast<F>(static_cast<uintptr_t>(k));
    else f = static_cast<F>(k);
}
template <typename F, size_t N> void put(int &k, F (&f)[N]) { for (F &e : f) put(k, e); }
template <typename... F> void number(F &...f) { int k = 0; (put(k, f), ...); }

void ordinals(wagg_plan_info &s) {
    auto &[a1, a2, a3, a4, a5, a6, a7, a8, a9, a10, a11, a12, a13, a14, a15, a16, a17, a18, a19] = s;
    number(a1, a2, a3, a4, a5, a6, a7, a8, a9, a10, a11, a12, a13, a14, a15, a16, a17, a18, a19);
}
void ordinals(wagg_dense_info &s) {
    auto &[a1, a2, a3, a4, a5, a6, a7, a8, a9, a10, a11, a12, a13, a14, a15, a16] = s;
    number(a1, a2, a3, a4, a5, a6, a7, a8, a9, a10, a11, a12, a13, a14, a15, a16);
}
void ordinals(wagg_host_stats &s) {
    auto &[a1, a2, a3, a4, a5, a6, a7, a8, a9, a10, a11, a12, a13, a14, a15, a16, a17, a18] = s;
    number(a1, a2, a3, a4, a5, a6, a7, a8, a9, a10, a11, a12, a13, a14, a15, a16, a17, a18);
}
void ordinals(wagg_apply_desc &s) {
    auto &[a1, a2, a3, a4, a5, a6, a7, a8, a9, a10, a11, a12, a13, a14, a15, a16, a17, a18, a19, a20, a21, a22, a23, a24, a25, a26, a27, a28, a29] = s;
    number(a1, a2, a3, a4, a5, a6, a7, a8, a9, a10, a11, a12, a13, a14, a15, a16, a17, a18, a19, a20, a21, a22, a23, a24, a25, a26, a27, a28, a29);
}
template <typename S> int fill_ordinals(void *out, uint64_t size) {
    S s;
    std::memset(&s, 0, sizeof(s));
    ordinals(s);
    copy_sized(out, size, &s, sizeof(s));
    return WAGG_OK;
}
}

void copy_sized(void *dst, uint64_t dst_size, const void *src, size_t src_size) {
    const size_t n = dst_size < src_size ? (size_t)dst_size : src_size;
    std::memcpy(dst, src, n);
    if (dst_size > src_size) std::memset(static_cast<char *>(dst) + src_size, 0, (size_t)(dst_size - src_size));
}
}

extern "C" int wagg_struct_size(int which) {
    switch (which) {
        case WAGG_STRUCT_PLAN_INFO: return (int)sizeof(wagg_plan_info);
        case WAGG_STRUCT_DENSE_INFO: return (int)sizeof(wagg_dense_info);
        case WAGG_STRUCT_HOST_STATS: return (int)sizeof(wagg_host_stats);
        case WAGG_STRUCT_APPLY_DESC: return (int)sizeof(wagg_apply_desc);
        default: wagg::set_error("wagg_struct_size: unknown struct id %d", which); return WAGG_EINVAL;
    }
}

extern "C" int wagg_struct_ordinals(int which, void *out, uint64_t size) {
    using namespace wagg;
    WAGG_REQUIRE(out != nullptr && size <= ((uint64_t)1 << 20), "wagg_struct_ordinals: NULL buffer or absurd size");
    switch (which) {
        case WAGG_STRUCT_PLAN_INFO: return fill_ordinals<wagg_plan_info>(out, size);
        case WAGG_STRUCT_DENSE_INFO: return fill_ordinals<wagg_dense_info>(out, size);
        case WAGG_STRUCT_HOST_STATS: return fill_ordinals<wagg_host_stats>(out, size);
        case WAGG_STRUCT_APPLY_DESC: return fill_ordinals<wagg_apply_desc>(out, size);
        default: set_error("wagg_struct_ordinals: unknown struct id %d", which); return WAGG_EINVAL;
    }
}
```

### climate_toolbox_amd/csrc/wagg_scratch.hip

```cpp
#include <mutex>
#include <new>
#include <vector>

#include "wagg_common.h"
#include "wagg_host.h"

namespace wagg {
namespace {
struct Block { int device; void *p; size_t cap; uint64_t tick; };
struct IdleStream { int device; hipStream_t st; int role; };
std::mutex g_mu;
std::vector<Block> g_free, g_live;
std::vector<IdleStream> g_streams;
uint64_t g_tick = 0;
constexpr size_t ROUND = (size_t)2 << 20;
constexpr size_t MAX_IDLE_STREAMS = 8;

size_t device_budget(int device) {
    static std::mutex mu;
    static std::vector<std::pair<int, size_t>> known;
    std::lock_guard<std::mutex> lock(mu);
    for (const auto &k : known) if (k.first == device) return k.second;
    size_t total = 0;
    hipDeviceProp_t prop;
    if (hipGetDeviceProperties(&prop, device) == hipSuccess) total = prop.totalGlobalMem;
    try { known.emplace_back(device, total / 16); } catch (const std::bad_alloc &) {}
    return total / 16;
}

void give_back(const std::vector<Block> &gone) {
    for (const Block &b : gone) note_cleanup(hipFree(b.p), "hipFree(kept scratch block)");
}
}

void release_scratch(int what) {
    std::vector<Block> blocks;
    std::vector<IdleStream> streams;
    {
        std::lock_guard<std::mutex> lock(g_mu);
        if (what & 1) blocks.swap(g_free);
        if (what & 2) streams.swap(g_streams);
    }
    give_back(blocks);
    for (const IdleStream &s : streams) note_cleanup(hipStreamDestroy(s.st), "hipStreamDestroy(kept stream)");
    if (what & 4) release_host_ring();
}

int64_t scratch_bytes_kept() {
    std::lock_guard<std::mutex> lock(g_mu);
    int64_t total = 0;
    for (const Block &b : g_free) total += (int64_t)b.cap;
    return total;
}

hipError_t scratch_alloc(void **out, size_t bytes) {
    *out = nullptr;
    int device = 0;
    hipError_t e = hipGetDevice(&device);
    if (e != hipSuccess) return e;
    const size_t need = (bytes + ROUND - 1) / ROUND * ROUND + (bytes == 0 ? ROUND : 0);
    const size_t slack = need / 4 > ((size_t)32 << 20) ? need / 4 : ((size_t)32 << 20);
    try {
        std::lock_guard<std::mutex> lock(g_mu);
        g_live.reserve(g_live.size() + 1);
        size_t best = g_free.size();
        for (size_t i = 0; i < g_free.size(); ++i)
            if (g_free[i].device == device && g_free[i].cap >= need && g_free[i].cap <= need + slack &&
                (best == g_free.size() || g_free[i].cap < g_free[best].cap))
                best = i;
        if (best != g_free.size()) {
            Block b = g_free[best];
            g_free.erase(g_free.begin() + (long)best);
            g_live.push_back(b);
            *out = b.p;
            return hipSuccess;
        }
    } catch (const std::bad_alloc &) {
        return hipErrorOutOfMemory;
    }
    void *p = nullptr;
    e = hipMalloc(&p, need);
    if (e == hipErrorOutOfMemory) {
        (void)hipGetLastError();
        release_scratch();
        e = hipMalloc(&p, need);
    }
    if (e != hipSuccess) return e;
    try {
        std::lock_guard<std::mutex> lock(g_mu);
        g_live.push_back(Block{device, p, need, 0});
    } catch (const std::bad_alloc &) {
        (void)hipFree(p);
        return hipErrorOutOfMemory;
    }
    *out = p;
    return hipSuccess;
}

void scratch_free(void *p, bool keep) {
    if (!p) return;
    std::vector<Block> gone;
    bool found = false;
    {
        std::lock_guard<std::mutex> lock(g_mu);
        for (size_t i = 0; i < g_live.size(); ++i) {
            if (g_live[i].p != p) continue;
            Block b = g_live[i];
            g_live.erase(g_live.begin() + (long)i);
            found = true;
            const size_t budget = device_budget(b.device);
            if (!keep || b.cap > budget) { gone.push_back(b); break; }
            b.tick = ++g_tick;
            try { g_free.push_back(b); } catch (const std::bad_alloc &) { gone.push_back(b); break; }
            size_t kept = 0;
            for (const Block &f : g_free) if (f.device == b.device) kept += f.cap;
            while (kept > budget) {
                size_t oldest = g_free.size();
                for (size_t k = 0; k < g_free.size(); ++k)
                    if (g_free[k].device == b.device && (oldest == g_free.size() || g_free[k].tick < g_free[oldest].tick)) oldest = k;
                if (oldest == g_free.size()) break;
                kept -= g_free[oldest].cap;
                try { gone.push_back(g_free[oldest]); } catch (const std::bad_alloc &) { break; }
                g_free.erase(g_free.begin() + (long)oldest);
            }
            break;
        }
    }
    if (!found) { note_cleanup(hipFree(p), "hipFree(block the scratch pool does not know)"); return; }
    give_back(gone);
}

hipError_t scratch_stream(hipStream_t *st, int role) {
    *st = nullptr;
    int device = 0;
// ... 39 lines not shown
```

### climate_toolbox_amd/csrc/wagg_util.hip

```cpp
#include <cstring>
#include <mutex>
#include <utility>

#include "wagg_common.h"
#include "wagg_host.h"

namespace wagg {

static thread_local char g_err[512] = "";

void clear_error() { g_err[0] = '\0'; }

void set_error(const char *fmt, ...) {
    va_list ap;
    va_start(ap, fmt);
    vsnprintf(g_err, sizeof(g_err), fmt, ap);
    va_end(ap);
}

hipError_t allow_dynamic_lds(const void *kern, size_t bytes) {
    static std::mutex mu;
    static std::vector<std::pair<const void *, int>> done;
    int dev = 0;
    hipError_t e = hipGetDevice(&dev);
// ... 252 lines not shown
    int64_t total = 1;
    for (int k = 0; k < 6; ++k) {
        d.shape[k] = k < nd ? shape[k] : 1; d.sstride[k] = k < nd ? sstride[k] : 0;
        WAGG_REQUIRE(d.shape[k] >= 0 && d.sstride[k] >= 0, "negative extent or stride");
        total *= d.shape[k];
    }
    if (total == 0) return WAGG_OK;
    WAGG_REQUIRE(src && dst, "NULL pointer");
    hipLaunchKernelGGL((relayout_kernel<T>), dim3(256 * 16), dim3(256), 0, (hipStream_t)stream, src, d, total, dst);
    WAGG_HIP(hipGetLastError());
    return WAGG_OK;
}

static int relayout_to_f64(const void *src, int src_type, int nd, const int64_t *shape, const int64_t *sstride, double *dst, void *stream) {
    WAGG_REQUIRE(nd >= 1 && nd <= 6 && shape && sstride, "1..6 dimensions");
    RelayoutDims d;
    d.nd = nd;
    int64_t total = 1;
    for (int k = 0; k < 6; ++k) {
        d.shape[k] = k < nd ? shape[k] : 1; d.sstride[k] = k < nd ? sstride[k] : 0;
        WAGG_REQUIRE(d.shape[k] >= 0 && d.sstride[k] >= 0, "negative extent or stride");
        total *= d.shape[k];
    }
    if (total == 0) return WAGG_OK;
    WAGG_REQUIRE(src && dst, "NULL pointer");
#define WAGG_TO_F64(S) hipLaunchKernelGGL((relayout_to_f64_kernel<S>), dim3(256 * 16), dim3(256), 0, (hipStream_t)stream, (const S *)src, d, total, dst)
    switch (src_type) {
        case WAGG_T_F16: WAGG_TO_F64(_Float16); break;
        case WAGG_T_BF16: WAGG_TO_F64(bf16_bits); break;
        case WAGG_T_I8: WAGG_TO_F64(int8_t); break;
        case WAGG_T_U8: WAGG_TO_F64(uint8_t); break;
        case WAGG_T_I16: WAGG_TO_F64(int16_t); break;
        case WAGG_T_I32: WAGG_TO_F64(int32_t); break;
        case WAGG_T_I64: WAGG_TO_F64(int64_t); break;
        case WAGG_T_F32: WAGG_TO_F64(float); break;
        case WAGG_T_F64: WAGG_TO_F64(double); break;
        default: WAGG_REQUIRE(false, "unknown element type %d", src_type);
    }
#undef WAGG_TO_F64
    WAGG_HIP(hipGetLastError());
    return WAGG_OK;
}
}

extern "C" int wagg_upload(void *dst_dev, const void *src_host, int64_t bytes) {
    using namespace wagg;
    clear_error();
    WAGG_REQUIRE(bytes >= 0 && (bytes == 0 || (dst_dev && src_host)), "bad upload request");
    return copy_to_device(dst_dev, src_host, (size_t)bytes, true);
}

extern "C" int wagg_relayout_to_f64(const void *src_dev, int src_type, int ndim, const int64_t *shape, const int64_t *src_strides,
                                    double *dst_dev, void *stream) {
    return wagg::relayout_to_f64(src_dev, src_type, ndim, shape, src_strides, dst_dev, stream);
}
extern "C" int wagg_combine_planes_f32(const float *planes_dev, int n_planes, int64_t plane_stride, const double *coefs,
                                       int64_t n, float *out_dev, void *stream) {
    return wagg::combine_planes<float>(planes_dev, n_planes, plane_stride, coefs, n, out_dev, stream);
}
extern "C" int wagg_combine_planes_f64(const double *planes_dev, int n_planes, int64_t plane_stride, const double *coefs,
                                       int64_t n, double *out_dev, void *stream) {
    return wagg::combine_planes<double>(planes_dev, n_planes, plane_stride, coefs, n, out_dev, stream);
}
extern "C" int wagg_take_axis(const void *src_dev, int64_t outer, int64_t n_src, int64_t inner_bytes, const int64_t *idx_dev,
                              int64_t n_idx, void *dst_dev, void *stream) {
    return wagg::take_axis(src_dev, outer, n_src, inner_bytes, idx_dev, n_idx, dst_dev, stream);
}
extern "C" int wagg_relayout_f32(const float *src_dev, int ndim, const int64_t *shape, const int64_t *src_strides, float *dst_dev,
                                 void *stream) {
    return wagg::relayout<float>(src_dev, ndim, shape, src_strides, dst_dev, stream);
}
extern "C" int wagg_relayout_f64(const double *src_dev, int ndim, const int64_t *shape, const int64_t *src_strides, double *dst_dev,
                                 void *stream) {
    return wagg::relayout<double>(src_dev, ndim, shape, src_strides, dst_dev, stream);
}

extern "C" int wagg_any_less_f32(const float *a, const float *b, int64_t n, int *result, void *stream) {
    return wagg::any_less<float>(a, b, n, result, stream);
}
extern "C" int wagg_any_less_f64(const double *a, const double *b, int64_t n, int *result, void *stream) {
    return wagg::any_less<double>(a, b, n, result, stream);
}

extern "C" int wagg_version(void) { return 10000 * 0 + 100 * 5 + 0; }

extern "C" int wagg_device_count(void) {
    int n = 0;
    if (hipGetDeviceCount(&n) != hipSuccess) return 0;
    return n;
}

extern "C" int wagg_shard_rows(int64_t T, int world, int rank, int64_t *start, int64_t *stop) {
    using namespace wagg;
    WAGG_REQUIRE(T >= 0 && world >= 1 && rank >= 0 && rank < world, "bad shard request: T=%lld world=%d rank=%d",
                 (long long)T, world, rank);
    WAGG_REQUIRE(start && stop, "NULL argument");
    const int64_t base = T / world, extra = T % world;
    *start = rank * base + (rank < extra ? rank : extra);
    *stop = *start + base + (rank < extra ? 1 : 0);
    return WAGG_OK;
}

extern "C" const char *wagg_last_error(void) { return wagg::g_err; }

extern "C" int wagg_gather_f32(const float *X, int64_t T, int64_t ldx, int layout,
                               const int32_t *cell_idx, int64_t nseg, float *out, int64_t ldo,
                               int out_layout, void *stream) {
    return wagg::gather<float>(X, T, ldx, layout, cell_idx, nseg, out, ldo, out_layout, stream);
}
extern "C" int wagg_gather_f64(const double *X, int64_t T, int64_t ldx, int layout,
                               const int32_t *cell_idx, int64_t nseg, double *out, int64_t ldo,
                               int out_layout, void *stream) {
    return wagg::gather<double>(X, T, ldx, layout, cell_idx, nseg, out, ldo, out_layout, stream);
}
extern "C" int wagg_synth_field_f32(float *X, int64_t T, int64_t G, int64_t ldx, uint32_t seed,
                                    float base, float amp, void *stream) {
    return wagg::synth_field<float>(X, T, G, ldx, seed, base, amp, stream);
}
extern "C" int wagg_synth_field_f64(double *X, int64_t T, int64_t G, int64_t ldx, uint32_t seed,
                                    double base, double amp, void *stream) {
    return wagg::synth_field<double>(X, T, G, ldx, seed, base, amp, stream);
}

extern "C" int wagg_profile_enable(int on) {
    using namespace wagg;
    if (on && !g_prof.created) {
        for (int i = 0; i < WAGG_PROFILE_SLOTS; ++i) {
            WAGG_HIP(hipEventCreate(&g_prof.a[i]));
            WAGG_HIP(hipEventCreate(&g_prof.b[i]));
        }
        g_prof.created = true;
    }
    g_prof.on = on != 0;
    g_prof.count = 0;
    return WAGG_OK;
}

namespace wagg { __global__ void empty_kernel() {} }

extern "C" int wagg_profile_event_overhead(void *stream, int n, float *median_ms, float *min_ms) {
    using namespace wagg;
    WAGG_REQUIRE(n >= 1 && n <= 256 && median_ms != nullptr, "n must be 1..256 and median_ms non-NULL");
    hipStream_t st = (hipStream_t)stream;
    std::vector<hipEvent_t> ev(2 * (size_t)n, nullptr);
    int rc = WAGG_OK;
    for (auto &e : ev)
        if (hipEventCreate(&e) != hipSuccess) { rc = WAGG_EHIP; break; }
    std::vector<float> ms;
    if (rc == WAGG_OK) {
        for (int i = 0; i < n + 8; ++i) {
            if (i < 8) hipLaunchKernelGGL(empty_kernel, dim3(1), dim3(64), 0, st);
            else hipExtLaunchKernelGGL(empty_kernel, dim3(1), dim3(64), 0u, st, ev[2 * (i - 8)], ev[2 * (i - 8) + 1], 0u);
        }
        if (hipStreamSynchronize(st) != hipSuccess || hipGetLastError() != hipSuccess) rc = WAGG_EHIP;
        for (int i = 0; rc == WAGG_OK && i < n; ++i) {
            float t = 0.f;
            if (hipEventElapsedTime(&t, ev[2 * i], ev[2 * i + 1]) != hipSuccess) rc = WAGG_EHIP;
            ms.push_back(t);
        }
    }
    for (auto e : ev) if (e) (void)hipEventDestroy(e);
    if (rc != WAGG_OK) { set_error("wagg_profile_event_overhead: a HIP call failed"); return rc; }
    std::sort(ms.begin(), ms.end());
    *median_ms = ms[ms.size() / 2];
    if (min_ms) *min_ms = ms[0];
    return WAGG_OK;
}
// ... 13 lines not shown
```

### climate_toolbox_amd/engine.py

```python
from __future__ import annotations

import ctypes as C
import threading

import numpy as np

from . import _lib
from ._lib import LAYOUT_GT, LAYOUT_TG, OUT_RT, OUT_TR, WaggError

_LAYOUTS = {"TG": LAYOUT_TG, "GT": LAYOUT_GT}
_OUTS = {"TR": OUT_TR, "RT": OUT_RT}


def require_gpu():
    L = _lib.load()
    if L.wagg_device_count() < 1:
        raise WaggError("no HIP device visible: the aggregation engine has no CPU fallback")
    import torch
    if not torch.cuda.is_available():
        raise WaggError("torch sees no GPU (needed for device buffers and streams)")
    return torch


class _on_device:
# ... 236 lines not shown
        L = _lib.load()
        levels = [(c, int(r)) for c, r in levels]
        keep, head, tail = _many_args(cell_idx, region_code, w_effs, levels)
        self._h = C.c_void_p()
        self._lease = threading.Lock()
        self.G, self.R = int(G), int(R)
        with _on_device(device):
            self.device = _current_device()
            _lib.check(L.wagg_plan_create_many(*head, self.G, self.R, int(row_len), tail[0], tail[1], tail[2], int(flags),
                                               C.byref(self._h)), "wagg_plan_create_many")
        del keep
        k, nl, oc = C.c_int(0), C.c_int(0), C.c_int64(0)
        lr = (C.c_int32 * 4)()
        _lib.check(L.wagg_plan_many_info(self._h, C.byref(k), C.byref(nl), lr, C.byref(oc)), "wagg_plan_many_info")
        self.n_weights, self.n_levels, self.out_cols = k.value, nl.value, int(oc.value)
        self.level_R = [self.R] + [int(lr[i]) for i in range(self.n_levels)]
        self.offsets = []
        off = 0
        for Rl in self.level_R:
            self.offsets.append([off + i * Rl for i in range(self.n_weights)])
            off += self.n_weights * Rl
        info = _lib.PlanInfo()
        _lib.check(L.wagg_plan_get_info_sized(self._h, C.byref(info), C.sizeof(info)), "wagg_plan_get_info_sized")
        self.info = {k: getattr(info, k) for k, _ in _lib.PlanInfo._fields_}
        self.info["nnz"] *= self.n_weights
        self.den = []
        for lv, Rl in enumerate(self.level_R):
            row = []
            for i in range(self.n_weights):
                d = np.empty(Rl, dtype=np.float64)
                _lib.check(L.wagg_plan_get_den_many(self._h, i, lv, _np_ptr(d, C.c_double)), "wagg_plan_get_den_many")
                row.append(d)
            self.den.append(row)

    def close(self):
        if getattr(self, "_h", None) is not None and self._h.value and _lib is not None and _lib._lib is not None:
            _lib._lib.wagg_plan_destroy(self._h)
            self._h = C.c_void_p()

    __del__ = close

    def status(self, stream=None):
        _lib.check(_lib.load().wagg_plan_status(self._h, _stream_handle(stream)), "wagg_plan_status")

    def split(self, full, out_layout="TR"):
        if out_layout == "TR":
            return [[full[:, o:o + Rl] for o in offs] for offs, Rl in zip(self.offsets, self.level_R)]
        return [[full[o:o + Rl] for o in offs] for offs, Rl in zip(self.offsets, self.level_R)]

    def apply(self, X, layout="TG", out_layout="TR", out=None, stream=None):
        import torch
        X = _check_X(X, layout)
        T = X.shape[0] if layout == "TG" else X.shape[1]
        if (X.shape[1] if layout == "TG" else X.shape[0]) != self.G:
            raise ValueError("X has the wrong number of grid cells (plan expects %d)" % self.G)
        shape = (T, self.out_cols) if out_layout == "TR" else (self.out_cols, T)
        if out is None:
            out = torch.empty(shape, dtype=X.dtype, device=X.device)
        elif tuple(out.shape) != shape or out.dtype != X.dtype or (shape[1] > 1 and out.stride(1) != 1):
            raise ValueError("out must be a %s %s tensor with contiguous rows" % (shape, X.dtype))
        _lib.run("wagg_apply (many)", plan_kind=_lib.PLAN_SEGMENT, plan=self._h, elem=_elem(X.dtype), source=_lib.SRC_DEVICE,
                 x=X.data_ptr(), T=T, ldx=_ld(X), layout=_LAYOUTS[layout], out=out.data_ptr(), ldo=_ld(out),
                 out_layout=_OUTS[out_layout], stream=_stream_handle(stream))
        return self.split(out, out_layout)

    def apply_host(self, X, flags=0, out=None, layout="TG", out_layout="TR"):
        X = np.ascontiguousarray(X)
        if X.dtype not in (np.float32, np.float64) or X.ndim != 2:
            raise TypeError("X must be a 2-D float32/float64 array")
        T = X.shape[0] if layout == "TG" else X.shape[1]
        shape = (T, self.out_cols) if out_layout == "TR" else (self.out_cols, T)
        out = _host_out(out, shape, X.dtype)
        with _on_device(self.device):
            _lib.run("wagg_apply (many, host)", plan_kind=_lib.PLAN_SEGMENT, plan=self._h, elem=_elem(X.dtype), source=_lib.SRC_HOST,
                     x=X.ctypes.data, T=T, ldx=X.shape[1], layout=_LAYOUTS[layout], out=out.ctypes.data, ldo=max(1, shape[1]),
                     out_layout=_OUTS[out_layout], flags=int(flags))
        return self.split(out, out_layout)


def _exact_flag(exact):
    return _lib.APPLY_EXACT_F32 if exact else 0


class DensePlan:

    def __init__(self, handle, G, R, device=None, recipe=None):
        self._h, self.G, self.R = handle, int(G), int(R)
        self.device = _current_device() if device is None else int(device)
        self._recipe = recipe
        self._lease = threading.Lock()
        den = np.empty(self.R, dtype=np.float64)
        _lib.check(_lib.load().wagg_dense_get_den(self._h, _np_ptr(den, C.c_double)), "wagg_dense_get_den")
        self.den = den
        inf = _lib.DenseInfo()
        _lib.check(_lib.load().wagg_dense_get_info_sized(self._h, C.byref(inf), C.sizeof(inf)), "wagg_dense_get_info_sized")
        self.info = {k: (float if ct is C.c_double else int)(getattr(inf, k)) for k, ct in _lib.DenseInfo._fields_}
        self.dtype = "float64" if self.info["elem_bytes"] == 8 else "float32"

    @staticmethod
    def _is64(dtype):
        return str(dtype).endswith("float64") or dtype is np.float64

    @classmethod
    def synth_blocklocal(cls, G, R, seed, fill=0.952, dtype="float32", device=None):
        require_gpu()
        h = C.c_void_p()
        L = _lib.load()
        fn = L.wagg_dense_create_synth_blocklocal_f64 if cls._is64(dtype) else L.wagg_dense_create_synth_blocklocal
        with _on_device(device):
            dev = _current_device()
            _lib.check(fn(int(G), int(R), int(seed), float(fill), C.byref(h)), "wagg_dense_create_synth_blocklocal")
        return cls(h, G, R, dev, (cls.synth_blocklocal, (G, R, seed), dict(fill=fill, dtype=dtype)))

    @classmethod
    def synth(cls, G, R, seed, fill=1.0, dtype="float32", device=None):
        require_gpu()
        h = C.c_void_p()
        L = _lib.load()
        fn = L.wagg_dense_create_synth_f64 if cls._is64(dtype) else L.wagg_dense_create_synth_sparse
        with _on_device(device):
            dev = _current_device()
            _lib.check(fn(int(G), int(R), int(seed), float(fill), C.byref(h)), "wagg_dense_create_synth")
        return cls(h, G, R, dev, (cls.synth, (G, R, seed), dict(fill=fill, dtype=dtype)))

    @classmethod
    def from_host(cls, W, device=None):
        require_gpu()
        W = np.asarray(W)
        h = C.c_void_p()
        with _on_device(device):
            dev = _current_device()
            if W.dtype == np.float64:
                W = np.ascontiguousarray(W)
                _lib.check(_lib.load().wagg_dense_create_host_f64(_np_ptr(W, C.c_double), W.shape[0], W.shape[1], C.byref(h)),
                           "wagg_dense_create_host_f64")
            else:
                W = np.ascontiguousarray(W, dtype=np.float32)
                _lib.check(_lib.load().wagg_dense_create_host(_np_ptr(W, C.c_float), W.shape[0], W.shape[1], C.byref(h)),
                           "wagg_dense_create_host")
        return cls(h, W.shape[0], W.shape[1], dev)

    @classmethod
    def from_segments(cls, cell_idx, region_code, w_eff, G, R, dtype="float32", device=None, form=None):
        require_gpu()
        ci = np.ascontiguousarray(cell_idx, dtype=np.int32)
        rc = np.ascontiguousarray(region_code, dtype=np.int32)
        we = np.ascontiguousarray(w_eff, dtype=np.float64)
        h = C.c_void_p()
        L = _lib.load()
        fn = L.wagg_dense_create_from_segments_f64 if cls._is64(dtype) else L.wagg_dense_create_from_segments
        with _on_device(device):
            dev = _current_device()
            _lib.check(fn(_np_ptr(ci, C.c_int32), _np_ptr(rc, C.c_int32), _np_ptr(we, C.c_double), len(ci), int(G),
                          int(R), _lib.FORCE_FORM[form], C.byref(h)), "wagg_dense_create_from_segments")
        return cls(h, G, R, dev)

    @classmethod
    def from_csr(cls, rowptr, col, val, G, R, dtype="float32", device=None, form=None, general_sort=False):
        require_gpu()
        rp = np.ascontiguousarray(rowptr, dtype=np.int64)
        co = np.ascontiguousarray(col, dtype=np.int32)
        va = np.ascontiguousarray(val, dtype=np.float64)
        if rp.shape != (int(G) + 1,) or co.shape != va.shape or co.ndim != 1 or (len(rp) and int(rp[-1]) != len(co)):
            raise ValueError("rowptr must hold G + 1 offsets ending at len(col) == len(val)")
        h = C.c_void_p()
        L = _lib.load()
        fn = L.wagg_dense_create_from_csr_f64 if cls._is64(dtype) else L.wagg_dense_create_from_csr
        with _on_device(device):
            dev = _current_device()
            _lib.check(fn(_np_ptr(rp, C.c_int64), _np_ptr(co, C.c_int32), _np_ptr(va, C.c_double), int(G), int(R),
                          _lib.FORCE_FORM[form] | (_lib.DENSE_GENERAL_SORT if general_sort else 0), C.byref(h)),
                       "wagg_dense_create_from_csr")
        return cls(h, G, R, dev)

    def replica(self, device):
        if self._recipe is not None:
            fn, args, kw = self._recipe
            return fn(*args, device=device, **kw)
        require_gpu()
        h = C.c_void_p()
        _lib.check(_lib.load().wagg_dense_clone(self._h, int(device), C.byref(h)), "wagg_dense_clone")
        return type(self)(h, self.G, self.R, int(device))

    def close(self):
        for r in getattr(self, "_replicas", {}).values():
            r.close()
        if getattr(self, "_h", None) is not None and self._h.value and _lib is not None and _lib._lib is not None:
            _lib._lib.wagg_dense_destroy(self._h)
            self._h = C.c_void_p()

    __del__ = close

    def _prep(self, X, out):
        import torch
        X = _check_X(X, "TG")
        want = torch.float64 if self.dtype == "float64" else torch.float32
        if X.dtype != want:
            raise TypeError("this dense plan serves %s data, got %s" % (self.dtype, X.dtype))
        if X.shape[1] != self.G:
            raise ValueError("X has %d grid cells, plan expects %d" % (X.shape[1], self.G))
        T = X.shape[0]
        if out is None:
            out = torch.empty((T, self.R), dtype=want, device=X.device)
        elif tuple(out.shape) != (T, self.R) or out.dtype != want or (self.R > 1 and out.stride(1) != 1):
            raise ValueError("out must be a (%d, %d) %s tensor with contiguous rows" % (T, self.R, self.dtype))
        return X, T, out

    def _run(self, what, **fields):
        _lib.run(what, plan_kind=_lib.PLAN_DENSE, elem=_elem(self.dtype), **fields)

    def apply(self, X, out=None, ksplit=0, stream=None, exact=False):
        X, T, out = self._prep(X, out)
        self._run("wagg_apply (dense)", plan=self._h, source=_lib.SRC_DEVICE, x=X.data_ptr(), T=T, ldx=_ld(X), out=out.data_ptr(),
                  ldo=_ld(out), ksplit=int(ksplit), stream=_stream_handle(stream), flags=_exact_flag(exact))
        return out

    def apply_poly(self, X, offset, power, out=None, ksplit=0, stream=None, exact=False):
        X, T, out = self._prep(X, out)
        self._run("wagg_apply (dense, poly)", plan=self._h, source=_lib.SRC_DEVICE, transform=_lib.XF_POLY, offset=float(offset),
                  pow_first=int(power), n_pow=1, x=X.data_ptr(), T=T, ldx=_ld(X), out=out.data_ptr(), ldo=_ld(out), ksplit=int(ksplit),
                  stream=_stream_handle(stream), flags=_exact_flag(exact))
        return out

    def apply_edd(self, tasmin, tasmax, threshold, offset=0.0, out=None, ksplit=0, stream=None, exact=False):
        tasmin, T, out = self._prep(tasmin, out)
        tasmax = _check_X(tasmax, "TG")
        if tasmax.shape != tasmin.shape or tasmax.dtype != tasmin.dtype or _ld(tasmax) != _ld(tasmin):
            raise ValueError("tasmin and tasmax must have the same shape, dtype and row stride")
        thr = (C.c_double * 1)(float(threshold))
        self._run("wagg_apply (dense, edd)", plan=self._h, source=_lib.SRC_DEVICE, transform=_lib.XF_EDD, offset=float(offset),
                  thresholds=thr, n_thr=1, x=tasmin.data_ptr(), x2=tasmax.data_ptr(), T=T, ldx=_ld(tasmin), out=out.data_ptr(),
                  ldo=_ld(out), ksplit=int(ksplit), stream=_stream_handle(stream), flags=_exact_flag(exact))
        return out

    def apply_host(self, X, flags=0, replicas=(), out=None, exact=False):
        flags = int(flags) & ~(_lib.HOST_LINES | _lib.HOST_LINES_WHOLE)
        want = np.float64 if self.dtype == "float64" else np.float32
        X = np.ascontiguousarray(X)
        if X.dtype != want or X.ndim != 2 or X.shape[1] != self.G:
            raise TypeError("X must be a (T, %d) %s array" % (self.G, self.dtype))
        out = _host_out(out, (X.shape[0], self.R), want)
        if replicas:
            plans = (self,) + tuple(replicas)
            hs = (C.c_void_p * len(plans))(*[p._h for p in plans])
            devs = (C.c_int32 * len(plans))(*[p.device for p in plans])
            self._run("wagg_apply (dense, host, multi-device)", plan=hs, n_plans=len(plans), devices=devs, source=_lib.SRC_HOST_MULTI,
                      x=X.ctypes.data, T=X.shape[0], ldx=X.shape[1], out=out.ctypes.data, ldo=max(1, self.R), flags=int(flags))
            return out
        with _on_device(self.device):
            self._run("wagg_apply (dense, host)", plan=self._h, source=_lib.SRC_HOST, x=X.ctypes.data, T=X.shape[0], ldx=X.shape[1],
                      out=out.ctypes.data, ldo=max(1, self.R), flags=int(flags) | _exact_flag(exact))
        return out

    def saw_inf(self, stream=None):
        saw = C.c_int(0)
        _lib.check(_lib.load().wagg_dense_saw_inf(self._h, _stream_handle(stream), C.byref(saw)), "wagg_dense_saw_inf")
        return bool(saw.value)


class ShardGroup:

    _TRANSPORTS = {"auto": _lib.GATHER_AUTO, "rccl": _lib.GATHER_RCCL, "peer": _lib.GATHER_PEER}

    def __init__(self, devices, transport="auto"):
        require_gpu()
        self.devices = [int(d) for d in devices]
        arr = (C.c_int32 * len(self.devices))(*self.devices)
        self._h = C.c_void_p()
        _lib.check(_lib.load().wagg_shard_group_create(arr, len(self.devices), self._TRANSPORTS[transport], C.byref(self._h)),
                   "wagg_shard_group_create")
        n, tr = C.c_int(0), C.c_int(0)
        _lib.check(_lib.load().wagg_shard_group_info(self._h, C.byref(n), C.byref(tr)), "wagg_shard_group_info")
        self.transport = {_lib.GATHER_RCCL: "rccl", _lib.GATHER_PEER: "peer"}[tr.value]

    def close(self):
        if getattr(self, "_h", None) is not None and self._h.value and _lib._lib is not None:
            _lib._lib.wagg_shard_group_destroy(self._h)
            self._h = C.c_void_p()

    __del__ = close

    def apply(self, plans, shards, root=0, out=None):
        import torch
        n = len(self.devices)
        if len(plans) != n or len(shards) != n:
            raise ValueError("the group has %d shards: need as many plans and tensors" % n)
        dense = isinstance(plans[0], DensePlan)
        if any(isinstance(p, DensePlan) != dense for p in plans):
            raise TypeError("all plans of a call are of one family")
        dtype = shards[0].dtype
        rows, lds = [], set()
        for i, x in enumerate(shards):
# ... 237 lines not shown
```

### include/wagg.h

```cpp
#ifndef WAGG_H
#define WAGG_H

#include <stdint.h>

#ifdef __cplusplus
extern "C" {
#endif

typedef enum wagg_status {
    WAGG_OK = 0,
    WAGG_EINVAL = -1,
    WAGG_EHIP = -2,
    WAGG_ENOMEM = -3,
    WAGG_ENODEV = -4,
    WAGG_EUNSUPPORTED = -5,
    WAGG_EKEY = -6,
    WAGG_EINTERNAL = -7
} wagg_status;

#define WAGG_LAYOUT_TG 0
#define WAGG_LAYOUT_GT 1
#define WAGG_OUT_TR 0
#define WAGG_OUT_RT 1

// ... 112 lines not shown
int wagg_apply_edd_f32(const wagg_plan *plan, const float *tasmin_dev, const float *tasmax_dev, int64_t T,
                       int64_t ldx, int layout, double offset, const double *thresholds, int n_thr,
                       float *out_dev, int64_t ldo, int64_t out_pstride, int out_layout, void *stream);
int wagg_apply_edd_f64(const wagg_plan *plan, const double *tasmin_dev, const double *tasmax_dev, int64_t T,
                       int64_t ldx, int layout, double offset, const double *thresholds, int n_thr,
                       double *out_dev, int64_t ldo, int64_t out_pstride, int out_layout, void *stream);
int wagg_apply_edd_host_f32(const wagg_plan *plan, const float *tasmin_host, const float *tasmax_host, int64_t T, int64_t ldx,
                            double offset, const double *thresholds, int n_thr, float *out_host, int64_t ldo,
                            int64_t out_pstride, int flags);
int wagg_apply_edd_host_f64(const wagg_plan *plan, const double *tasmin_host, const double *tasmax_host, int64_t T, int64_t ldx,
                            double offset, const double *thresholds, int n_thr, double *out_host, int64_t ldo,
                            int64_t out_pstride, int flags);

int wagg_transform_poly_f32(const float *X_dev, int64_t n, double offset, int power, float *out_dev, void *stream);
int wagg_transform_poly_f64(const double *X_dev, int64_t n, double offset, int power, double *out_dev, void *stream);
int wagg_transform_edd_f32(const float *tasmin_dev, const float *tasmax_dev, int64_t n, double offset,
                           const double *coefs, const double *thresholds, int n_terms, float *out_dev, void *stream);
int wagg_transform_edd_f64(const double *tasmin_dev, const double *tasmax_dev, int64_t n, double offset,
                           const double *coefs, const double *thresholds, int n_terms, double *out_dev, void *stream);
int wagg_combine_planes_f32(const float *planes_dev, int n_planes, int64_t plane_stride, const double *coefs, int64_t n,
                            float *out_dev, void *stream);
int wagg_combine_planes_f64(const double *planes_dev, int n_planes, int64_t plane_stride, const double *coefs, int64_t n,
                            double *out_dev, void *stream);
int wagg_take_axis(const void *src_dev, int64_t outer, int64_t n_src, int64_t inner_bytes, const int64_t *idx_dev,
                   int64_t n_idx, void *dst_dev, void *stream);
int wagg_relayout_f32(const float *src_dev, int ndim, const int64_t *shape, const int64_t *src_strides, float *dst_dev, void *stream);
int wagg_relayout_f64(const double *src_dev, int ndim, const int64_t *shape, const int64_t *src_strides, double *dst_dev, void *stream);
#define WAGG_T_F16 0
#define WAGG_T_BF16 1
#define WAGG_T_I8 2
#define WAGG_T_U8 3
#define WAGG_T_I16 4
#define WAGG_T_I32 5
#define WAGG_T_I64 6
#define WAGG_T_F32 7
#define WAGG_T_F64 8
int wagg_relayout_to_f64(const void *src_dev, int src_type, int ndim, const int64_t *shape, const int64_t *src_strides,
                         double *dst_dev, void *stream);
int wagg_upload(void *dst_dev, const void *src_host, int64_t bytes);
int wagg_any_less_f32(const float *a_dev, const float *b_dev, int64_t n, int *result, void *stream);
int wagg_any_less_f64(const double *a_dev, const double *b_dev, int64_t n, int *result, void *stream);

int wagg_gather_f32(const float *X_dev, int64_t T, int64_t ldx, int layout,
                    const int32_t *cell_idx_dev, int64_t nseg, float *out_dev, int64_t ldo,
                    int out_layout, void *stream);
int wagg_gather_f64(const double *X_dev, int64_t T, int64_t ldx, int layout,
                    const int32_t *cell_idx_dev, int64_t nseg, double *out_dev, int64_t ldo,
                    int out_layout, void *stream);

int wagg_dense_create_synth(int64_t G, int32_t R, uint32_t seed, wagg_dense **out);
int wagg_dense_create_synth_sparse(int64_t G, int32_t R, uint32_t seed, double fill, wagg_dense **out);
int wagg_dense_create_host(const float *W_host, int64_t G, int32_t R, wagg_dense **out);
#define WAGG_DENSE_FORM_AUTO 0
#define WAGG_DENSE_FORCE_FULL 1
#define WAGG_DENSE_FORCE_TILES 2
#define WAGG_DENSE_FORCE_ENTRIES 3
#define WAGG_DENSE_GENERAL_SORT 16
int wagg_dense_create_from_segments(const int32_t *cell_idx, const int32_t *region_code,
                                    const double *w_eff, int64_t nseg, int64_t G, int32_t R,
                                    int flags, wagg_dense **out);
int wagg_dense_create_from_csr(const int64_t *rowptr, const int32_t *col, const double *val, int64_t G, int32_t R,
                               int flags, wagg_dense **out);
int wagg_dense_create_synth_blocklocal(int64_t G, int32_t R, uint32_t seed, double fill, wagg_dense **out);
#define WAGG_FORM_FULL 0
#define WAGG_FORM_TILES 1
#define WAGG_FORM_ENTRIES 2
int wagg_dense_create_synth_f64(int64_t G, int32_t R, uint32_t seed, double fill, wagg_dense **out);
int wagg_dense_create_host_f64(const double *W_host, int64_t G, int32_t R, wagg_dense **out);
int wagg_dense_create_from_segments_f64(const int32_t *cell_idx, const int32_t *region_code,
                                        const double *w_eff, int64_t nseg, int64_t G, int32_t R,
                                        int flags, wagg_dense **out);
int wagg_dense_create_from_csr_f64(const int64_t *rowptr, const int32_t *col, const double *val, int64_t G, int32_t R,
                                   int flags, wagg_dense **out);
int wagg_dense_create_synth_blocklocal_f64(int64_t G, int32_t R, uint32_t seed, double fill, wagg_dense **out);
typedef struct wagg_dense_info {
    int64_t G, n_tiles, w_bytes;
    int32_t R, n_kt, n_nt, tiled;
    int32_t form, elem_bytes;
    int64_t nnz;
    double build_s, build_upload_s;
    double est_row_s[3];
    int64_t walked_entries;
    int32_t one_pass_sort, reserved0;
} wagg_dense_info;
int wagg_dense_get_info(const wagg_dense *d, wagg_dense_info *info);
int wagg_dense_get_info_sized(const wagg_dense *d, void *info, uint64_t size);
int wagg_release_scratch(void);
int64_t wagg_scratch_bytes(void);
int wagg_dense_clone(const wagg_dense *src, int device, wagg_dense **out);
int wagg_dense_destroy(wagg_dense *d);
int wagg_dense_get_den(const wagg_dense *d, double *den_host );
int wagg_dense_apply_f32(wagg_dense *d, const float *X_dev, int64_t T, int64_t ldx,
                         float *out_dev, int64_t ldo, int ksplit, void *stream);
int wagg_dense_apply_f64(wagg_dense *d, const double *X_dev, int64_t T, int64_t ldx,
                         double *out_dev, int64_t ldo, int ksplit, void *stream);
int wagg_dense_apply_poly_f32(wagg_dense *d, const float *X_dev, int64_t T, int64_t ldx, double offset,
                              int power, float *out_dev, int64_t ldo, int ksplit, void *stream);
int wagg_dense_apply_edd_f32(wagg_dense *d, const float *tasmin_dev, const float *tasmax_dev, int64_t T,
                             int64_t ldx, double offset, double threshold, float *out_dev, int64_t ldo,
                             int ksplit, void *stream);
int wagg_dense_apply_poly_f64(wagg_dense *d, const double *X_dev, int64_t T, int64_t ldx, double offset,
                              int power, double *out_dev, int64_t ldo, int ksplit, void *stream);
int wagg_dense_apply_edd_f64(wagg_dense *d, const double *tasmin_dev, const double *tasmax_dev, int64_t T,
                             int64_t ldx, double offset, double threshold, double *out_dev, int64_t ldo,
                             int ksplit, void *stream);
int wagg_dense_apply_host_f32(wagg_dense *d, const float *X_host, int64_t T, int64_t ldx,
                              float *out_host, int64_t ldo, int flags);
int wagg_dense_apply_host_f64(wagg_dense *d, const double *X_host, int64_t T, int64_t ldx,
                              double *out_host, int64_t ldo, int flags);
int wagg_dense_apply_host_multi_f32(wagg_dense *const *plans, const int *devices, int n_devices, const float *X_host,
                                    int64_t T, int64_t ldx, float *out_host, int64_t ldo, int flags);
int wagg_dense_apply_host_multi_f64(wagg_dense *const *plans, const int *devices, int n_devices, const double *X_host,
                                    int64_t T, int64_t ldx, double *out_host, int64_t ldo, int flags);
int wagg_dense_saw_inf(wagg_dense *d, void *stream, int *saw);

int wagg_synth_table_csr(int64_t G, int32_t R, uint32_t seed, double fill, int blocklocal, int64_t *rowptr_host,
                         int32_t *col_host, double *val_host, int64_t capacity, int64_t *nnz_out);
int wagg_synth_field_f32(float *X_dev, int64_t T, int64_t G, int64_t ldx, uint32_t seed,
                         float base, float amp, void *stream);
int wagg_synth_field_f64(double *X_dev, int64_t T, int64_t G, int64_t ldx, uint32_t seed,
                         double base, double amp, void *stream);

typedef struct wagg_shard_group wagg_shard_group;
#define WAGG_GATHER_AUTO 0
#define WAGG_GATHER_RCCL 1
#define WAGG_GATHER_PEER 2
int wagg_shard_group_create(const int *devices, int n, int transport, wagg_shard_group **out);
int wagg_shard_group_destroy(wagg_shard_group *g);
int wagg_shard_group_info(const wagg_shard_group *g, int *n_shards, int *transport );
int wagg_apply_sharded_f32(wagg_shard_group *g, const wagg_plan *const *plans, const float *const *X_dev, const int64_t *rows,
                           int64_t ldx, float *out_root, int64_t ldo, int root);
int wagg_apply_sharded_f64(wagg_shard_group *g, const wagg_plan *const *plans, const double *const *X_dev, const int64_t *rows,
                           int64_t ldx, double *out_root, int64_t ldo, int root);
int wagg_dense_apply_sharded_f32(wagg_shard_group *g, wagg_dense *const *plans, const float *const *X_dev, const int64_t *rows,
                                 int64_t ldx, float *out_root, int64_t ldo, int root);
int wagg_dense_apply_sharded_f64(wagg_shard_group *g, wagg_dense *const *plans, const double *const *X_dev, const int64_t *rows,
                                 int64_t ldx, double *out_root, int64_t ldo, int root);

#define WAGG_PLAN_SEGMENT 0
#define WAGG_PLAN_DENSE 1
#define WAGG_SRC_DEVICE 0
#define WAGG_SRC_HOST 1
#define WAGG_SRC_HOST_MULTI 2
#define WAGG_SRC_SHARDED 3
#define WAGG_XF_NONE 0
#define WAGG_XF_POLY 1
#define WAGG_XF_EDD 2
#define WAGG_APPLY_EXACT_F32 0x10000
typedef struct wagg_apply_desc {
    uint64_t struct_size;
    int32_t plan_kind, elem, source, transform;
    const void *plan;
    const void *x, *x2;
    void *out;
    int64_t T, ldx, ldo, out_pstride;
    int32_t layout, out_layout;
    double offset;
    int32_t pow_first, n_pow;
    const double *thresholds;
    int32_t n_thr, flags;
    int32_t ksplit, n_plans;
    const int32_t *devices;
    const int64_t *rows;
    void *group;
    int32_t root, reserved0;
    void *stream;
} wagg_apply_desc;
int wagg_apply(const wagg_apply_desc *desc);

int wagg_plan_create_many(const int32_t *cell_idx, const int32_t *region_code, const double *const *w_eff, int n_weights,
                          int64_t nseg, int64_t G, int32_t R, int64_t row_len, const int32_t *const *level_code,
                          const int32_t *level_R, int n_levels, int flags, wagg_plan **out);
int wagg_plan_many_info(const wagg_plan *plan, int *n_weights, int *n_levels, int32_t *level_R, int64_t *out_cols);
// ... 7 lines not shown
```

Measured before the change: 235500 billion.

## Cache presplit fp16 hi/lo weight tiles for dense split kernel

Adds a one-time presplit kernel that converts the f32 weight tiles into fp16 hi/lo pairs and keeps them in a per-plan device buffer. The split MFMA kernel then loads the ready fp16 fragments directly instead of running the split per tile, and a double-buffered register rotation unrolls the tile loop by two. The cost is the same amount of extra device memory as the weights, managed by a free-memory check, a limit knob and plan-cache eviction hooks. It also adds a hipMemGetInfo and capture-status check on the path that decides whether to build the buffer.

```diff
diff --git a/climate_toolbox_amd/_lib.py b/climate_toolbox_amd/_lib.py
--- a/climate_toolbox_amd/_lib.py
+++ b/climate_toolbox_amd/_lib.py
@@ -43,6 +43,7 @@
     "wagg_apply", "wagg_struct_size", "wagg_struct_ordinals", "wagg_plan_get_info_sized", "wagg_dense_get_info_sized",
     "wagg_host_stats_read_sized",
     "wagg_plan_create_many", "wagg_plan_many_info", "wagg_plan_get_den_many",
+    "wagg_dense_presplit_limit", "wagg_dense_release_presplit",
 )
 STRUCT_PLAN_INFO, STRUCT_DENSE_INFO, STRUCT_HOST_STATS, STRUCT_APPLY_DESC = 0, 1, 2, 3
 PLAN_SEGMENT, PLAN_DENSE = 0, 1
@@ -78,7 +79,7 @@
                 ("form", C.c_int32), ("elem_bytes", C.c_int32), ("nnz", C.c_int64),
                 ("build_s", C.c_double), ("build_upload_s", C.c_double),
                 ("est_full_s", C.c_double), ("est_tiles_s", C.c_double), ("est_entries_s", C.c_double), ("walked_entries", C.c_int64),
-                ("one_pass_sort", C.c_int32), ("reserved0", C.c_int32)]
+                ("one_pass_sort", C.c_int32), ("reserved0", C.c_int32), ("presplit_bytes", C.c_int64)]
 
 
 class WaggError(RuntimeError):
@@ -218,6 +219,8 @@
     L.wagg_dense_create_synth_sparse.argtypes = [C.c_int64, C.c_int32, C.c_uint32, C.c_double, C.POINTER(vp)]
     L.wagg_dense_get_info.argtypes = [vp, C.POINTER(DenseInfo)]
     L.wagg_dense_destroy.argtypes = [vp]
+    L.wagg_dense_presplit_limit.argtypes = [C.c_int64]
+    L.wagg_dense_release_presplit.argtypes = [vp]
     L.wagg_dense_clone.argtypes = [vp, C.c_int, C.POINTER(vp)]
     L.wagg_release_scratch.argtypes = []
     L.wagg_scratch_bytes.argtypes = []
diff --git a/climate_toolbox_amd/_plans.py b/climate_toolbox_amd/_plans.py
--- a/climate_toolbox_amd/_plans.py
+++ b/climate_toolbox_amd/_plans.py
@@ -95,12 +95,26 @@
 
 
 def _plan_bytes(plan):
-    return int(plan.info.get("w_bytes", 0)) if isinstance(plan, DensePlan) else 16 * int(plan.info.get("nnz", 0))
+    if isinstance(plan, DensePlan):
+        info = plan.info
+        return int(info.get("w_bytes", 0)) + int(info.get("presplit_bytes", 0))
+    return 16 * int(plan.info.get("nnz", 0))
 
 
 def _evict_plans(byte_budget, keep):
     freed = 0
     held = sum(_plan_bytes(p) for p in _PLAN_CACHE.values())
+    for old in list(_PLAN_CACHE.values()):
+        if not (len(_PLAN_CACHE) > keep or held > max(byte_budget, 0)):
+            break
+        b = int(old.info.get("presplit_bytes", 0)) if isinstance(old, DensePlan) else 0
+        if b and old._lease.acquire(blocking=False):
+            try:
+                old.release_presplit()
+            finally:
+                old._lease.release()
+            held -= b
+            freed += b
     for key in list(_PLAN_CACHE):
         if not (len(_PLAN_CACHE) > keep or held > max(byte_budget, 0)):
             break
diff --git a/climate_toolbox_amd/csrc/wagg_common.h b/climate_toolbox_amd/csrc/wagg_common.h
--- a/climate_toolbox_amd/csrc/wagg_common.h
+++ b/climate_toolbox_amd/csrc/wagg_common.h
@@ -147,6 +147,9 @@
 hipError_t scratch_stream(hipStream_t *st, int role = 0);
 void scratch_stream_done(hipStream_t st, int role = 0, bool keep = true);
 void release_scratch(int what = 7);
+int64_t scratch_bytes_kept(int device = -1);
+void note_device_release();
+uint64_t device_release_count();
 template <typename T>
 struct ScratchBuf {
     T *p = nullptr;
@@ -164,9 +167,10 @@
     DevBuf() = default;
     DevBuf(const DevBuf &) = delete;
     DevBuf &operator=(const DevBuf &) = delete;
-    ~DevBuf() { if (p) (void)hipFree(p); }
+    ~DevBuf() { release(); }
+    void release() { if (p) { (void)hipFree(p); p = nullptr; n = 0; note_device_release(); } }
     hipError_t alloc(size_t count) {
-        if (p) { (void)hipFree(p); p = nullptr; }
+        release();
         n = count;
         hipError_t e = hipMalloc((void **)&p, (count ? count : 1) * sizeof(T));
         if (e == hipErrorOutOfMemory) {
diff --git a/climate_toolbox_amd/csrc/wagg_dense.hip b/climate_toolbox_amd/csrc/wagg_dense.hip
--- a/climate_toolbox_amd/csrc/wagg_dense.hip
+++ b/climate_toolbox_amd/csrc/wagg_dense.hip
@@ -1,4 +1,5 @@
 #include <algorithm>
+#include <atomic>
 #include <cfloat>
 #include <chrono>
 #include <cmath>
@@ -773,8 +774,8 @@
 #undef WAGG_PICK
 }
 
-static const void *pick_split_kernel(int MT) {
-#define WAGG_PICK(M) case M: return (const void *)dense_split_kernel<M>
+static const void *pick_split_kernel(int MT, bool pre) {
+#define WAGG_PICK(M) case M: return pre ? (const void *)dense_split_kernel<M, 0, true> : (const void *)dense_split_kernel<M>
     switch (MT) {
         WAGG_PICK(1); WAGG_PICK(2); WAGG_PICK(3); WAGG_PICK(4); WAGG_PICK(5); WAGG_PICK(6); WAGG_PICK(8);
         WAGG_PICK(10); WAGG_PICK(12); WAGG_PICK(14); WAGG_PICK(16); WAGG_PICK(18); WAGG_PICK(20);
@@ -782,6 +783,40 @@
         default: return nullptr;
     }
 #undef WAGG_PICK
+}
+
+static std::atomic<int64_t> g_presplit_limit{-1};
+
+static bool presplit_ready(wagg_dense *d, hipStream_t st) {
+    if (d->wsplit.p) return true;
+    const int64_t limit = g_presplit_limit.load(std::memory_order_relaxed);
+    const int64_t bytes = d->w_slots() * 16;
+    if (limit == 0 || (limit > 0 && bytes > limit) || bytes <= 0) return false;
+    const uint64_t epoch = device_release_count();
+    if (d->presplit_short >= 0 && epoch == d->presplit_epoch && ++d->presplit_skipped % 64 != 0) return false;
+    hipStreamCaptureStatus cap = hipStreamCaptureStatusNone;
+    if (hipStreamIsCapturing(st, &cap) != hipSuccess) { (void)hipGetLastError(); return false; }
+    if (cap != hipStreamCaptureStatusNone) return false;
+    size_t free_b = 0, total_b = 0;
+    if (hipMemGetInfo(&free_b, &total_b) != hipSuccess) { (void)hipGetLastError(); return false; }
+    const int64_t avail = (int64_t)free_b + scratch_bytes_kept(d->device);
+    auto too_short = [&]() { d->presplit_short = avail; d->presplit_epoch = epoch; return false; };
+    if (d->presplit_short >= 0 && avail <= d->presplit_short) return too_short();
+    if (avail < bytes + (int64_t)(total_b / 16)) return too_short();
+    if (d->wsplit.alloc((size_t)d->w_slots() * 4) != hipSuccess) {
+        (void)hipGetLastError();
+        d->wsplit.release();
+        return too_short();
+    }
+    const int64_t n_items = d->n_tiles * 1024;
+    const int64_t nblk = (n_items + 255) / 256 < (int64_t)d->ncu * 32 ? (n_items + 255) / 256 : (int64_t)d->ncu * 32;
+    hipLaunchKernelGGL(dense_presplit_kernel, dim3((unsigned)nblk), dim3(256), 0, st, reinterpret_cast<const f32x4 *>(d->W.p),
+                       (const float *)d->wmax.p, d->n_kt, n_items, reinterpret_cast<u32x4 *>(d->wsplit.p));
+    hipError_t e = hipGetLastError();
+    if (e == hipSuccess) e = hipStreamSynchronize(st);
+    if (e != hipSuccess) { d->wsplit.release(); return too_short(); }
+    d->presplit_short = -1;
+    return true;
 }
 
 static int dense_apply_split(wagg_dense *d, const float *X_dev, int64_t Tn, int64_t ldx, const PackXfT<float> &xf,
@@ -790,8 +825,7 @@
     const int kt_per_slice = (n_kt + S - 1) / S;
     const int64_t nblk = (int64_t)n_nt * n_mb * S;
     WAGG_REQUIRE(nblk < (int64_t)0x7fffffff, "grid too large");
-    const void *kern = pick_split_kernel(MT);
-    if (!kern) { set_error("no split kernel for MT=%d", MT); return WAGG_EINVAL; }
+    if (!pick_split_kernel(MT, false)) { set_error("no split kernel for MT=%d", MT); return WAGG_EINVAL; }
     const size_t need = (size_t)nblk * bm * D_BN;
     if (d->slabs.n < need) WAGG_HIP(d->slabs.alloc(need));
     const int64_t x_slots = (int64_t)n_mb * n_kt * bm * 8;
@@ -799,8 +833,14 @@
     if (d->xmax.n < (size_t)Tn) WAGG_HIP(d->xmax.alloc((size_t)Tn));
     const int aligned = ((ldx * sizeof(float)) % 16 == 0) && ((reinterpret_cast<uintptr_t>(X_dev) & 15) == 0) &&
                         (xf.mode != XF_EDD || (reinterpret_cast<uintptr_t>(xf.X2) & 15) == 0);
+    bool want_pre = true;
 #ifdef WAGG_DIAG
-    if (const char *dbg = MT == D_MT ? getenv("WAGG_SPLIT_DBG") : nullptr) {
+    if (const char *dbg = getenv("WAGG_SPLIT_DBG")) want_pre = !strcmp(dbg, "pre");
+#endif
+    const bool pre = want_pre && presplit_ready(d, st);
+    const void *kern = pick_split_kernel(MT, pre);
+#ifdef WAGG_DIAG
+    if (const char *dbg = MT == D_MT && !pre ? getenv("WAGG_SPLIT_DBG") : nullptr) {
         switch (atoi(dbg)) {
             case 1: kern = (const void *)dense_split_kernel<D_MT, 1>; break;
             case 4: kern = (const void *)dense_split_kernel<D_MT, 4>; break;
@@ -821,7 +861,7 @@
                        (const unsigned *)xmax, reinterpret_cast<f16x8 *>(d->xp.p), xf, d->inf_dev);
     WAGG_HIP(hipGetLastError());
     const f16x8 *xp = reinterpret_cast<const f16x8 *>(d->xp.p);
-    const float *wp = d->W.p, *wmax = d->wmax.p;
+    const float *wp = pre ? d->wsplit.p : d->W.p, *wmax = d->wmax.p;
     float *slabs = d->slabs.p;
     int n_kt_a = n_kt, n_nt_a = n_nt, n_mb_a = n_mb, S_a = S, kps = kt_per_slice;
     void *args[] = {&xp, &wp, &wmax, &n_kt_a, &n_nt_a, &n_mb_a, &S_a, &kps, &slabs};
@@ -1050,6 +1090,7 @@
     info->walked_entries = d->walked_entries;
     info->one_pass_sort = d->one_pass_sort ? 1 : 0;
     info->reserved0 = 0;
+    info->presplit_bytes = d->wsplit.p ? d->w_slots() * 16 : 0;
     copy_sized(info_buf, size, &st, sizeof(st));
     return WAGG_OK;
 }
@@ -1120,6 +1161,24 @@
     return WAGG_OK;
 }
 
+extern "C" int wagg_dense_presplit_limit(int64_t bytes) {
+    using namespace wagg;
+    clear_error();
+    WAGG_REQUIRE(bytes >= -1, "the limit is -1 (automatic), 0 (never) or a byte count");
+    g_presplit_limit.store(bytes, std::memory_order_relaxed);
+    note_device_release();
+    return WAGG_OK;
+}
+
+extern "C" int wagg_dense_release_presplit(wagg_dense *d) {
+    using namespace wagg;
+    clear_error();
+    WAGG_REQUIRE(d != nullptr, "dense plan is NULL");
+    d->wsplit.release();
+    d->presplit_short = -1;
+    return WAGG_OK;
+}
+
 extern "C" int wagg_dense_destroy(wagg_dense *d) {
     delete d;
     return WAGG_OK;
diff --git a/climate_toolbox_amd/csrc/wagg_dense_int.h b/climate_toolbox_amd/csrc/wagg_dense_int.h
--- a/climate_toolbox_amd/csrc/wagg_dense_int.h
+++ b/climate_toolbox_amd/csrc/wagg_dense_int.h
@@ -63,6 +63,10 @@
     wagg::DevBuf<float> W, den32, slabs, xp;
     wagg::DevBuf<double> den64;
     wagg::DevBuf<float> wmax, xmax;
+    wagg::DevBuf<float> wsplit;
+    int64_t presplit_short = -1;
+    uint64_t presplit_epoch = 0;
+    unsigned presplit_skipped = 0;
     std::vector<double> den_host;
     bool tiled = false;
     int64_t n_tiles = 0;
diff --git a/climate_toolbox_amd/csrc/wagg_dense_split.inc b/climate_toolbox_amd/csrc/wagg_dense_split.inc
--- a/climate_toolbox_amd/csrc/wagg_dense_split.inc
+++ b/climate_toolbox_amd/csrc/wagg_dense_split.inc
@@ -36,7 +36,7 @@
     return __builtin_amdgcn_make_buffer_rsrc(reinterpret_cast<void *>(u), (short)0, bytes, 0x00020000);
 }
 
-template <int MT, int DBG = 0>
+template <int MT, int DBG = 0, bool PRE = false>
 __global__ __launch_bounds__(D_THREADS, 2) void dense_split_kernel(
     const f16x8 *__restrict__ Xp, const float *__restrict__ Wp, const float *__restrict__ wmax, int n_kt, int n_nt, int n_mb,
     int S, int kt_per_slice, float *__restrict__ slabs) {
@@ -62,8 +62,8 @@
     const int kt1 = kt0 + kt_per_slice < n_kt ? kt0 + kt_per_slice : n_kt;
     const int ntiles = kt1 > kt0 ? kt1 - kt0 : 0;
     const int64_t w_first = (int64_t)nt * n_kt + kt0;
-    const int ew0 = split_exp(wmax[nt * D_BN + wave * 32 + lr]);
-    const int ew1 = split_exp(wmax[nt * D_BN + wave * 32 + 16 + lr]);
+    const int ew0 = PRE ? 0 : split_exp(wmax[nt * D_BN + wave * 32 + lr]);
+    const int ew1 = PRE ? 0 : split_exp(wmax[nt * D_BN + wave * 32 + 16 + lr]);
 
     const int f = lr >> 1;
     const unsigned frag0 = (lr * 8 + (kq ^ f)) * 16;
@@ -98,14 +98,25 @@
         b11 = __builtin_bit_cast(f32x4, __builtin_amdgcn_raw_buffer_load_b128(wr_, wfrag1 + 2048, 0, 0)); \
     } while (0)
 
+#define WAGG_LOAD_WP(tile, H0, L0, H1, L1)                                                        \
+    do {                                                                                          \
+        const auto wr_ = WAGG_RSRC(wslice + (int64_t)(tile) * D_WTB, D_WTB);                      \
+        H0 = __builtin_bit_cast(f16x8, __builtin_amdgcn_raw_buffer_load_b128(wr_, wfrag0, 0, 0));         \
+        L0 = __builtin_bit_cast(f16x8, __builtin_amdgcn_raw_buffer_load_b128(wr_, wfrag1, 0, 0));         \
+        H1 = __builtin_bit_cast(f16x8, __builtin_amdgcn_raw_buffer_load_b128(wr_, wfrag0 + 2048, 0, 0));  \
+        L1 = __builtin_bit_cast(f16x8, __builtin_amdgcn_raw_buffer_load_b128(wr_, wfrag1 + 2048, 0, 0));  \
+    } while (0)
+
     f32x4 acc[MT][2];
 #pragma unroll
     for (int m = 0; m < MT; ++m) acc[m][0] = acc[m][1] = f32x4{0, 0, 0, 0};
 
     f32x4 b00, b01, b10, b11;
+    f16x8 pAh0, pAl0, pAh1, pAl1, pBh0, pBl0, pBh1, pBl1;
     if (ntiles > 0) {
         const int t1 = ntiles > 1 ? 1 : 0;
-        WAGG_LOAD_W(0);
+        if constexpr (PRE) WAGG_LOAD_WP(0, pAh0, pAl0, pAh1, pAl1);
+        else WAGG_LOAD_W(0);
         WAGG_DMA_XALL(0, 0);
         WAGG_DMA_XALL(t1, 1);
         asm volatile("s_waitcnt vmcnt(0)" ::: "memory");
@@ -158,53 +169,74 @@
     } while (0)
 
     int bcur = 0;
-    for (int tile = 0; tile < ntiles; ++tile) {
-        const char *img = lds + bcur * XT4;
-        const int bfar = bcur == 0 ? 2 : bcur - 1;
-        const int tnext = tile + 1 < ntiles ? tile + 1 : ntiles - 1;
-        const int tfar = tile + 2 < ntiles ? tile + 2 : ntiles - 1;
-        const auto xfar = WAGG_RSRC(xslice + (int64_t)tfar * XT4, XT4);
-        f16x8 wh0, wl0, wh1, wl1, aAh, aAl, aBh, aBl;
-        WAGG_READ_A(aAh, aAl, 0);
-        WAGG_SPLIT(b00, b01, ew0, wh0, wl0);
-        if constexpr (MT > 1) WAGG_READ_A(aBh, aBl, MT > 1 ? 1 : 0);
-        __builtin_amdgcn_sched_barrier(0);
-        WAGG_MFMA16(0, 0, aAh, wl0);
-        WAGG_MFMA16(0, 0, aAl, wh0);
-        WAGG_MFMA16(0, 0, aAh, wh0);
-        if constexpr (MT > 1) {
-            WAGG_MFMA16(MT > 1 ? 1 : 0, 0, aBh, wl0);
-            WAGG_MFMA16(MT > 1 ? 1 : 0, 0, aBl, wh0);
-            WAGG_MFMA16(MT > 1 ? 1 : 0, 0, aBh, wh0);
+#define WAGG_TILE(CH0, CL0, CH1, CL1, NH0, NL0, NH1, NL1)                                         \
+    do {                                                                                          \
+        const char *img = lds + bcur * XT4;                                                       \
+        const int bfar = bcur == 0 ? 2 : bcur - 1;                 \
+        const int tnext = tile + 1 < ntiles ? tile + 1 : ntiles - 1;    \
+        const int tfar = tile + 2 < ntiles ? tile + 2 : ntiles - 1;                               \
+        const auto xfar = WAGG_RSRC(xslice + (int64_t)tfar * XT4, XT4);                           \
+        f16x8 wh0, wl0, wh1, wl1, aAh, aAl, aBh, aBl;                                             \
+         \
+        WAGG_READ_A(aAh, aAl, 0);                                                                 \
+        if constexpr (PRE) { wh0 = CH0; wl0 = CL0; wh1 = CH1; wl1 = CL1; }                        \
+        else WAGG_SPLIT(b00, b01, ew0, wh0, wl0);                                                 \
+        if constexpr (MT > 1) WAGG_READ_A(aBh, aBl, MT > 1 ? 1 : 0);                              \
+        __builtin_amdgcn_sched_barrier(0);                                                        \
+        WAGG_MFMA16(0, 0, aAh, wl0);                                                              \
+        WAGG_MFMA16(0, 0, aAl, wh0);                                                              \
+        WAGG_MFMA16(0, 0, aAh, wh0);                                                              \
+        if constexpr (MT > 1) {                                                                   \
+            WAGG_MFMA16(MT > 1 ? 1 : 0, 0, aBh, wl0);                                             \
+            WAGG_MFMA16(MT > 1 ? 1 : 0, 0, aBl, wh0);                                             \
+            WAGG_MFMA16(MT > 1 ? 1 : 0, 0, aBh, wh0);                                             \
+        }                                                                                         \
+        if constexpr (!PRE) WAGG_SPLIT(b10, b11, ew1, wh1, wl1);                                  \
+        __builtin_amdgcn_sched_barrier(0);                                                        \
+        if constexpr (!(DBG & 1)) {                                                               \
+            if constexpr (PRE) WAGG_LOAD_WP(tnext, NH0, NL0, NH1, NL1);                           \
+            else WAGG_LOAD_W(tnext);                                                              \
+        }                                                                                         \
+        __builtin_amdgcn_sched_barrier(0);                                                        \
+        WAGG_MFMA16(0, 1, aAh, wl1);                                                              \
+        WAGG_MFMA16(0, 1, aAl, wh1);                                                              \
+        WAGG_MFMA16(0, 1, aAh, wh1);                                                              \
+        __builtin_amdgcn_sched_barrier(0);                                                        \
+        if constexpr (MT > 2) WAGG_READ_A(aAh, aAl, MT > 2 ? 2 : 0);                              \
+        __builtin_amdgcn_sched_barrier(0);                                                        \
+        if constexpr (MT > 1) {                                                                   \
+            WAGG_MFMA16(MT > 1 ? 1 : 0, 1, aBh, wl1);                                             \
+            WAGG_MFMA16(MT > 1 ? 1 : 0, 1, aBl, wh1);                                             \
+            WAGG_MFMA16(MT > 1 ? 1 : 0, 1, aBh, wh1);                                             \
+        }                                                                                         \
+        __builtin_amdgcn_sched_barrier(0);                                                        \
+        WAGG_DMA_BLOCK(0); WAGG_DMA_BLOCK(1);                                                     \
+        WAGG_BLOCK(2); WAGG_BLOCK(3); WAGG_BLOCK(4); WAGG_BLOCK(5);                               \
+        WAGG_BLOCK(6); WAGG_BLOCK(7); WAGG_BLOCK(8); WAGG_BLOCK(9); WAGG_BLOCK(10); WAGG_BLOCK(11); \
+        WAGG_BLOCK(12); WAGG_BLOCK(13); WAGG_BLOCK(14); WAGG_BLOCK(15); WAGG_BLOCK(16); WAGG_BLOCK(17); \
+        WAGG_BLOCK(18); WAGG_BLOCK(19); WAGG_BLOCK(20); WAGG_BLOCK(21); WAGG_BLOCK(22);           \
+        static_assert(MT <= 23, "row blocks are written out up to 22");                           \
+        __builtin_amdgcn_sched_barrier(0);                                                        \
+        if constexpr (!(DBG & 4)) {                                                               \
+            __builtin_amdgcn_s_waitcnt(WAIT_TILE);                                                \
+            __builtin_amdgcn_s_barrier();                                                         \
+        }                                                                                         \
+        bcur = bcur == 2 ? 0 : bcur + 1;                                                          \
+    } while (0)
+    if constexpr (PRE) {
+        int tile = 0;
+        if (ntiles & 1) {
+            WAGG_TILE(pAh0, pAl0, pAh1, pAl1, pBh0, pBl0, pBh1, pBl1);
+            pAh0 = pBh0; pAl0 = pBl0; pAh1 = pBh1; pAl1 = pBl1;
+            tile = 1;
         }
-        WAGG_SPLIT(b10, b11, ew1, wh1, wl1);
-        __builtin_amdgcn_sched_barrier(0);
-        if constexpr (!(DBG & 1)) WAGG_LOAD_W(tnext);
-        __builtin_amdgcn_sched_barrier(0);
-        WAGG_MFMA16(0, 1, aAh, wl1);
-        WAGG_MFMA16(0, 1, aAl, wh1);
-        WAGG_MFMA16(0, 1, aAh, wh1);
-        __builtin_amdgcn_sched_barrier(0);
-        if constexpr (MT > 2) WAGG_READ_A(aAh, aAl, MT > 2 ? 2 : 0);
-        __builtin_amdgcn_sched_barrier(0);
-        if constexpr (MT > 1) {
-            WAGG_MFMA16(MT > 1 ? 1 : 0, 1, aBh, wl1);
-            WAGG_MFMA16(MT > 1 ? 1 : 0, 1, aBl, wh1);
-            WAGG_MFMA16(MT > 1 ? 1 : 0, 1, aBh, wh1);
+        for (; tile < ntiles; ++tile) {
+            WAGG_TILE(pAh0, pAl0, pAh1, pAl1, pBh0, pBl0, pBh1, pBl1);
+            ++tile;
+            WAGG_TILE(pBh0, pBl0, pBh1, pBl1, pAh0, pAl0, pAh1, pAl1);
         }
-        __builtin_amdgcn_sched_barrier(0);
-        WAGG_DMA_BLOCK(0); WAGG_DMA_BLOCK(1);
-        WAGG_BLOCK(2); WAGG_BLOCK(3); WAGG_BLOCK(4); WAGG_BLOCK(5);
-        WAGG_BLOCK(6); WAGG_BLOCK(7); WAGG_BLOCK(8); WAGG_BLOCK(9); WAGG_BLOCK(10); WAGG_BLOCK(11);
-        WAGG_BLOCK(12); WAGG_BLOCK(13); WAGG_BLOCK(14); WAGG_BLOCK(15); WAGG_BLOCK(16); WAGG_BLOCK(17);
-        WAGG_BLOCK(18); WAGG_BLOCK(19); WAGG_BLOCK(20); WAGG_BLOCK(21); WAGG_BLOCK(22);
-        static_assert(MT <= 23, "row blocks are written out up to 22");
-        __builtin_amdgcn_sched_barrier(0);
-        if constexpr (!(DBG & 4)) {
-            __builtin_amdgcn_s_waitcnt(WAIT_TILE);
-            __builtin_amdgcn_s_barrier();
-        }
-        bcur = bcur == 2 ? 0 : bcur + 1;
+    } else {
+        for (int tile = 0; tile < ntiles; ++tile) WAGG_TILE(pAh0, pAl0, pAh1, pAl1, pBh0, pBl0, pBh1, pBl1);
     }
     asm volatile("s_waitcnt vmcnt(0)" ::: "memory");
 
@@ -220,6 +252,8 @@
 #undef WAGG_DMA_X
 #undef WAGG_DMA_XALL
 #undef WAGG_LOAD_W
+#undef WAGG_LOAD_WP
+#undef WAGG_TILE
 #undef WAGG_DMA_AT
 #undef WAGG_DMA_BLOCK
 #undef WAGG_SPLIT
@@ -227,6 +261,21 @@
 #undef WAGG_READ_A
 #undef WAGG_BLOCK_
 #undef WAGG_BLOCK
+}
+
+__global__ void dense_presplit_kernel(const f32x4 *__restrict__ Wp, const float *__restrict__ wmax, int n_kt, int64_t n_items,
+                                      u32x4 *__restrict__ Ws) {
+    const int64_t stride = (int64_t)gridDim.x * blockDim.x;
+    for (int64_t s = (int64_t)blockIdx.x * blockDim.x + threadIdx.x; s < n_items; s += stride) {
+        const int64_t tile = s >> 10;
+        const int row = (int)(s >> 2) & 255, p = (int)s & 3;
+        const int nt = (int)(tile / n_kt);
+        const int64_t i0 = tile * D_WSLOTS + tile_slot(row, p), i1 = tile * D_WSLOTS + tile_slot(row, p + 4);
+        f16x8 hi, lo;
+        split_w8(Wp[i0], Wp[i1], split_exp(wmax[nt * D_BN + row]), hi, lo);
+        Ws[i0] = __builtin_bit_cast(u32x4, hi);
+        Ws[i1] = __builtin_bit_cast(u32x4, lo);
+    }
 }
 
 __global__ void dense_rowmax_kernel(const float *__restrict__ X, int64_t ldx, int64_t G, PackXfT<float> xf,
diff --git a/climate_toolbox_amd/csrc/wagg_desc.hip b/climate_toolbox_amd/csrc/wagg_desc.hip
--- a/climate_toolbox_amd/csrc/wagg_desc.hip
+++ b/climate_toolbox_amd/csrc/wagg_desc.hip
@@ -388,8 +388,8 @@
     number(a1, a2, a3, a4, a5, a6, a7, a8, a9, a10, a11, a12, a13, a14, a15, a16, a17, a18, a19);
 }
 void ordinals(wagg_dense_info &s) {
-    auto &[a1, a2, a3, a4, a5, a6, a7, a8, a9, a10, a11, a12, a13, a14, a15, a16] = s;
-    number(a1, a2, a3, a4, a5, a6, a7, a8, a9, a10, a11, a12, a13, a14, a15, a16);
+    auto &[a1, a2, a3, a4, a5, a6, a7, a8, a9, a10, a11, a12, a13, a14, a15, a16, a17] = s;
+    number(a1, a2, a3, a4, a5, a6, a7, a8, a9, a10, a11, a12, a13, a14, a15, a16, a17);
 }
 void ordinals(wagg_host_stats &s) {
     auto &[a1, a2, a3, a4, a5, a6, a7, a8, a9, a10, a11, a12, a13, a14, a15, a16, a17, a18] = s;
diff --git a/climate_toolbox_amd/csrc/wagg_scratch.hip b/climate_toolbox_amd/csrc/wagg_scratch.hip
--- a/climate_toolbox_amd/csrc/wagg_scratch.hip
+++ b/climate_toolbox_amd/csrc/wagg_scratch.hip
@@ -1,3 +1,4 @@
+#include <atomic>
 #include <mutex>
 #include <new>
 #include <vector>
@@ -30,8 +31,13 @@
 
 void give_back(const std::vector<Block> &gone) {
     for (const Block &b : gone) note_cleanup(hipFree(b.p), "hipFree(kept scratch block)");
+    if (!gone.empty()) note_device_release();
 }
+std::atomic<uint64_t> g_releases{0};
 }
+
+void note_device_release() { g_releases.fetch_add(1, std::memory_order_relaxed); }
+uint64_t device_release_count() { return g_releases.load(std::memory_order_relaxed); }
 
 void release_scratch(int what) {
     std::vector<Block> blocks;
@@ -46,10 +52,10 @@
     if (what & 4) release_host_ring();
 }
 
-int64_t scratch_bytes_kept() {
+int64_t scratch_bytes_kept(int device) {
     std::lock_guard<std::mutex> lock(g_mu);
     int64_t total = 0;
-    for (const Block &b : g_free) total += (int64_t)b.cap;
+    for (const Block &b : g_free) if (device < 0 || b.device == device) total += (int64_t)b.cap;
     return total;
 }
 
diff --git a/climate_toolbox_amd/csrc/wagg_util.hip b/climate_toolbox_amd/csrc/wagg_util.hip
--- a/climate_toolbox_amd/csrc/wagg_util.hip
+++ b/climate_toolbox_amd/csrc/wagg_util.hip
@@ -358,7 +358,7 @@
     return wagg::any_less<double>(a, b, n, result, stream);
 }
 
-extern "C" int wagg_version(void) { return 10000 * 0 + 100 * 5 + 0; }
+extern "C" int wagg_version(void) { return 10000 * 0 + 100 * 6 + 0; }
 
 extern "C" int wagg_device_count(void) {
     int n = 0;
diff --git a/climate_toolbox_amd/engine.py b/climate_toolbox_amd/engine.py
--- a/climate_toolbox_amd/engine.py
+++ b/climate_toolbox_amd/engine.py
@@ -342,6 +342,10 @@
     return _lib.APPLY_EXACT_F32 if exact else 0
 
 
+def presplit_limit(nbytes=-1):
+    _lib.check(_lib.load().wagg_dense_presplit_limit(int(nbytes)), "wagg_dense_presplit_limit")
+
+
 class DensePlan:
 
     def __init__(self, handle, G, R, device=None, recipe=None):
@@ -352,10 +356,19 @@
         den = np.empty(self.R, dtype=np.float64)
         _lib.check(_lib.load().wagg_dense_get_den(self._h, _np_ptr(den, C.c_double)), "wagg_dense_get_den")
         self.den = den
+        self.info = {}
+        self._refresh_info()
+        self.dtype = "float64" if self.info["elem_bytes"] == 8 else "float32"
+
+    def _refresh_info(self):
         inf = _lib.DenseInfo()
         _lib.check(_lib.load().wagg_dense_get_info_sized(self._h, C.byref(inf), C.sizeof(inf)), "wagg_dense_get_info_sized")
-        self.info = {k: (float if ct is C.c_double else int)(getattr(inf, k)) for k, ct in _lib.DenseInfo._fields_}
-        self.dtype = "float64" if self.info["elem_bytes"] == 8 else "float32"
+        self.info.update({k: (float if ct is C.c_double else int)(getattr(inf, k)) for k, ct in _lib.DenseInfo._fields_})
+
+    def release_presplit(self):
+        if self._h is not None and self._h.value:
+            _lib.check(_lib.load().wagg_dense_release_presplit(self._h), "wagg_dense_release_presplit")
+            self._refresh_info()
 
     @staticmethod
     def _is64(dtype):
@@ -468,6 +481,7 @@
 
     def _run(self, what, **fields):
         _lib.run(what, plan_kind=_lib.PLAN_DENSE, elem=_elem(self.dtype), **fields)
+        self._refresh_info()
 
     def apply(self, X, out=None, ksplit=0, stream=None, exact=False):
         X, T, out = self._prep(X, out)
diff --git a/include/wagg.h b/include/wagg.h
--- a/include/wagg.h
+++ b/include/wagg.h
@@ -218,6 +218,7 @@
     double est_row_s[3];
     int64_t walked_entries;
     int32_t one_pass_sort, reserved0;
+    int64_t presplit_bytes;
 } wagg_dense_info;
 int wagg_dense_get_info(const wagg_dense *d, wagg_dense_info *info);
 int wagg_dense_get_info_sized(const wagg_dense *d, void *info, uint64_t size);
@@ -225,6 +226,8 @@
 int64_t wagg_scratch_bytes(void);
 int wagg_dense_clone(const wagg_dense *src, int device, wagg_dense **out);
 int wagg_dense_destroy(wagg_dense *d);
+int wagg_dense_presplit_limit(int64_t bytes);
+int wagg_dense_release_presplit(wagg_dense *d);
 int wagg_dense_get_den(const wagg_dense *d, double *den_host );
 int wagg_dense_apply_f32(wagg_dense *d, const float *X_dev, int64_t T, int64_t ldx,
                          float *out_dev, int64_t ldo, int ksplit, void *stream);
```

Measured after the change: 242700 billion, median of 6. 1.03x the previous value.
